# zhang-xuan1314/ABC-Net

Hardware: AMD Instinct MI355X
Metric: training images/sec (384x384, b16/GPU) (higher is better)
Workload: dtype bf16; 1 GPU; unet.py train step (pack+fwd+fused loss+bwd+allreduce+Adam), 384x384, batch 16/GPU, dropout 0.2; global_batch=16, parallelism=dp1, graph=True, device_meters=False, device_rasteriser=False, device_extraction=False, logits_stored=True

## Files before the change

abc-net_amd/_lib.py:

```python
from __future__ import annotations

import ctypes as C
import os

_HERE = os.path.dirname(os.path.abspath(__file__))
LIB_PATH = os.path.join(_HERE, "libabcnet_hip.so")

F32, BF16, FP8 = 0, 1, 2
MAX_TAPS = 49
OMEGA_RAW, OMEGA_PEAKS = 0, 1

vp, i32, u32, i64, f32, f64 = C.c_void_p, C.c_int32, C.c_uint32, C.c_int64, C.c_float, C.c_double


class ActSrc(C.Structure):
    _fields_ = [("x", vp), ("scale", vp), ("shift", vp), ("slope", vp), ("Hx", i32), ("Wx", i32), ("ldx", i32),
                ("pool", i32), ("drop_p", f32), ("drop_seed", u32), ("planar", i32), ("ctot", i32), ("drop_salt", vp)]


class ConvDesc(C.Structure):
    _fields_ = [("src", ActSrc), ("w", vp), ("bias", vp), ("y", vp), ("stats", vp),
                ("dtype_in", i32), ("dtype_c", i32), ("dtype_out", i32),
                ("B", i32), ("Hin", i32), ("Win", i32), ("cin_off", i32), ("Cin", i32), ("Hg", i32), ("Wg", i32),
                ("Hout", i32), ("Wout", i32), ("ldy", i32), ("cout_off", i32), ("Cout", i32), ("Cout_pad", i32),
                ("stride", i32), ("om", i32), ("oy0", i32), ("ox0", i32), ("ntaps", i32),
                ("tap_dy", C.c_int8 * MAX_TAPS), ("tap_dx", C.c_int8 * MAX_TAPS), ("stats_rows", i32), ("accumulate", i32),
                ("planar_out", i32), ("ctot_out", i32), ("out_act", i32), ("out_slope", f32), ("pool_y", vp), ("ld_pool", i32),
                ("stem_x", vp), ("stem_w", vp), ("stem_scale", vp), ("stem_bias", vp), ("stem_slope", f32),
                ("out_scale", vp), ("out_quant", vp), ("out_quant_stride", i32), ("heads_epi", vp),
                ("actbwd_y", vp), ("actbwd_ld", i32), ("actbwd_coff", i32), ("actbwd_scale", vp), ("actbwd_shift", vp), ("actbwd_slope", vp),
                ("actbwd_mean", vp), ("actbwd_invstd", vp), ("head_aux", vp), ("head_aux_mode", i32)]


class HeadsEpi(C.Structure):
    _fields_ = [("w2", vp), ("bias", vp), ("oscale", vp), ("y", vp), ("Cout", i32), ("Cout_pad", i32)]


class PackDesc(C.Structure):
    _fields_ = [("w", vp), ("dst", vp), ("mode", i32), ("dtype_c", i32), ("Cout", i32), ("Cin", i32), ("kh", i32),
                ("kw", i32), ("py", i32), ("px", i32), ("rows_pad", i32), ("red_pad", i32), ("red_total", i32),
                ("red_off", i32), ("ck", i32), ("rows_total", i32), ("rows_off", i32), ("layout", i32), ("row_scale", vp)]


class BnFwdDesc(C.Structure):
    _fields_ = [("partial", vp), ("nblk", i32), ("C", i32), ("count", f64), ("rows", i32), ("gamma", vp), ("beta", vp),
                ("scale", vp), ("shift", vp), ("mean", vp), ("invstd", vp), ("running_mean", vp), ("running_var", vp),
                ("num_batches_tracked", vp), ("eps", f32), ("momentum", f32)]


class ActBwdDesc(C.Structure):
    _fields_ = [("y_raw", vp), ("ld_y", i32), ("dA_same", vp), ("ld_same", i32), ("dA_pool", vp), ("ld_pool", i32),
                ("g", vp), ("ld_g", i32), ("partial", vp), ("scale", vp), ("shift", vp), ("slope", vp), ("mean", vp),
                ("invstd", vp), ("dtype", i32), ("B", i32), ("H", i32), ("W", i32), ("C", i32), ("cy_off", i32),
                ("csame_off", i32), ("cpool_off", i32), ("drop_p", f32), ("drop_seed", u32), ("drop_ld", i32), ("drop_salt", vp)]


class BnBwdDesc(C.Structure):
    _fields_ = [("partial", vp), ("nblk", i32), ("C", i32), ("count", f64), ("gamma", vp), ("invstd", vp),
                ("dgamma", vp), ("dbeta", vp), ("k1", vp), ("k2", vp), ("gscale", vp),
                ("mean", vp), ("ca", vp), ("cb", vp), ("cc", vp), ("in_scale", vp)]


class BnApplyDesc(C.Structure):
    _fields_ = [("g", vp), ("ld_g", i32), ("y_raw", vp), ("ld_y", i32), ("cy_off", i32), ("mean", vp), ("invstd", vp),
                ("k1", vp), ("k2", vp), ("gscale", vp), ("dtype", i32), ("C", i32), ("npix", i64), ("out", vp), ("ld_out", i32)]


class WgradDesc(C.Structure):
    _fields_ = [("p", ActSrc), ("q", ActSrc), ("partial", vp), ("dtype_p", i32), ("dtype_q", i32), ("dtype_c", i32),
                ("B", i32), ("Hg", i32), ("Wg", i32), ("Hq", i32), ("Wq", i32), ("cp_off", i32), ("Ca", i32),
                ("cq_off", i32), ("Cb", i32), ("stride", i32), ("ntaps", i32), ("nsplit", i32),
                ("tap_dy", C.c_int8 * MAX_TAPS), ("tap_dx", C.c_int8 * MAX_TAPS),
                ("p2", vp), ("ld_p2", i32), ("cp2_off", i32), ("p_dual", i32), ("p_out", vp), ("ld_pout", i32),
                ("rowsum_partial", vp)]


class WgradReduceDesc(C.Structure):
    _fields_ = [("partial", vp), ("nsplit", i32), ("ntaps", i32), ("Ca", i32), ("Cb", i32), ("Ca_pad", i32),
                ("Cb_pad", i32), ("dw", vp), ("accumulate", i32)]


class LossDesc(C.Structure):
    _fields_ = [("logits", vp * 8), ("dlogits", vp * 8), ("t_atom", vp), ("t_types", vp), ("t_charges", vp),
                ("t_hs", vp), ("t_bond", vp), ("t_btypes", vp), ("t_rho", vp), ("t_omega", vp), ("B", i32), ("h", i32),
                ("w", i32), ("partial", vp)]


class LossFinDesc(C.Structure):
    _fields_ = [("partial", vp), ("nblk", i32), ("s", vp), ("ds", vp), ("out", vp), ("chan_scale", vp), ("nchan", i32),
                ("chan_off", i32 * 8), ("head_c", i32 * 8), ("grad_scale", f32)]


class AdamDesc(C.Structure):
    _fields_ = [("p", vp), ("g", vp), ("m", vp), ("v", vp), ("n", i64), ("step", vp), ("lr", f32), ("beta1", f32),
                ("beta2", f32), ("eps", f32), ("weight_decay", f32), ("grad_scale", f32)]


class LossScaleDesc(C.Structure):
    _fields_ = [("dlogits", vp * 8), ("n", i64 * 8), ("head_scale", vp), ("ds", vp), ("grad_out", vp)]


ADAM_MAX_CLASSES = 32


class AdamSeg(C.Structure):
    _fields_ = [("p", vp), ("g", vp), ("m", vp), ("v", vp), ("n", i64), ("first_chunk", i64), ("cls", i32), ("pad_", i32)]


class AdamClass(C.Structure):
    _fields_ = [("step_size", f32), ("bc2_sqrt", f32), ("beta1", f32), ("beta2", f32), ("eps", f32), ("weight_decay", f32),
                ("pad_", f32 * 2)]


class AdamMultiDesc(C.Structure):
    _fields_ = [("segs", vp), ("nseg", i32), ("nclass", i32), ("chunk_total", i64), ("cls", AdamClass * ADAM_MAX_CLASSES)]


class NmsDesc(C.Structure):
    _fields_ = [("atom", vp), ("bond", vp), ("rho", vp), ("omega", vp), ("B", i32), ("h", i32), ("w", i32),
                ("n_omega", i32), ("atom_mask", vp), ("bond_mask", vp), ("rho_abs", vp), ("omega_mask", vp)]


class CbamChannelDesc(C.Structure):
    _fields_ = [("partial", vp), ("tiles_per_img", i32), ("B", i32), ("C", i32), ("mid", i32), ("HW", f64), ("scale", vp),
                ("shift", vp), ("w1", vp), ("b1", vp), ("w2", vp), ("b2", vp), ("ca", vp), ("avgz", vp), ("maxz", vp),
                ("hid_avg", vp), ("hid_max", vp), ("dw1", vp), ("db1", vp), ("dw2", vp), ("db2", vp), ("d_avgz", vp),
                ("d_maxz", vp), ("work", vp), ("ext", vp), ("first", vp)]


class CbamPixDesc(C.Structure):
    _fields_ = [("y", vp), ("ld_y", i32), ("cy_off", i32), ("scale", vp), ("shift", vp), ("mean", vp), ("invstd", vp),
                ("ca", vp), ("maxz", vp), ("d_avgz", vp), ("d_maxz", vp), ("sa", vp), ("st", vp), ("amax", vp), ("du", vp),
                ("dst", vp), ("res", vp), ("ld_res", i32), ("cres_off", i32), ("res_pool", i32), ("out", vp), ("ld_out", i32),
                ("cout_off", i32), ("d_same", vp), ("ld_same", i32), ("csame_off", i32), ("d_pool", vp), ("ld_pool", i32),
                ("cpool_off", i32), ("g", vp), ("ld_g", i32), ("dz", vp), ("ld_dz", i32), ("partial", vp), ("dtype", i32),
                ("B", i32), ("H", i32), ("W", i32), ("C", i32), ("ext", vp), ("first", vp)]


class CbamConv7Desc(C.Structure):
    _fields_ = [("st", vp), ("w7", vp), ("b7", vp), ("sa", vp), ("du", vp), ("dst", vp), ("dw_partial", vp), ("dw7", vp),
                ("db7", vp), ("B", i32), ("H", i32), ("W", i32)]


class MetricsDesc(C.Structure):
    _fields_ = [("logits", vp * 8), ("t_atom", vp), ("t_types", vp), ("t_charges", vp), ("t_hs", vp), ("t_bond", vp),
                ("t_btypes", vp), ("t_rho", vp), ("t_omega", vp), ("B", i32), ("h", i32), ("w", i32), ("peaks", vp),
                ("partial", vp), ("totals", vp), ("last", vp)]


class ExtractDesc(C.Structure):
    _fields_ = [("atom_mask", vp), ("bond_mask", vp), ("types", vp), ("charges", vp), ("hs", vp), ("btypes", vp), ("rho", vp),
                ("omega", vp), ("B", i32), ("h", i32), ("w", i32), ("cap_atoms", i32), ("cap_bonds", i32), ("counts", vp),
                ("atoms", vp), ("bonds", vp), ("bond_rho", vp), ("work", vp), ("work_masks", vp), ("btype_idx", vp),
                ("omega_rule", i32)]


class RasterDesc(C.Structure):
    _fields_ = [("t_atom", vp), ("t_types", vp), ("t_charges", vp), ("t_hs", vp), ("t_bond", vp), ("t_btypes", vp), ("t_rho", vp),
                ("t_omega", vp), ("B", i32), ("h", i32), ("w", i32), ("max_atoms", i32), ("max_bonds", i32), ("atoms", vp),
                ("n_atoms", vp), ("bonds", vp), ("n_bonds", vp), ("rho", vp), ("group_flags", vp), ("prev_atoms", vp), ("prev_bonds", vp),
                ("prev_rho", vp), ("prev_counts", vp), ("incremental", i32)]


class HeadsFusedDesc(C.Structure):
    _fields_ = [("feat", vp), ("ld", i32), ("scale", vp), ("shift", vp), ("slope", vp), ("mean", vp), ("invstd", vp),
                ("drop_p", f32), ("drop_seed", u32), ("drop_salt", vp), ("w2", vp * 8), ("b2", vp * 8), ("w2_pack", vp),
                ("logits", vp * 8), ("t_atom", vp), ("t_types", vp), ("t_charges", vp), ("t_hs", vp), ("t_bond", vp),
                ("t_btypes", vp), ("t_rho", vp), ("t_omega", vp), ("dl", vp), ("g", vp), ("bn_partial", vp), ("loss_partial", vp),
                ("B", i32), ("h", i32), ("w", i32), ("chan_scale", vp), ("chan_off", i32 * 8), ("dw2", vp * 8), ("db2", vp * 8),
                ("wgrad_work", vp), ("keep_mask", vp), ("target_flags", vp), ("zero_bytes", vp)]


class ConvTDesc(C.Structure):
    _fields_ = [("src", ActSrc), ("w", vp), ("bias", vp), ("y", vp), ("dtype", i32), ("B", i32), ("Hin", i32), ("Win", i32), ("cin_off", i32),
                ("Cin", i32), ("Hout", i32), ("Wout", i32), ("ldy", i32), ("cout_off", i32), ("Cout", i32), ("Cout_pad", i32)]


class ImageDesc(C.Structure):
    _fields_ = [("out", vp), ("src", vp), ("src_stride", i64), ("src_pitch", i32), ("src_max_h", i32), ("params", vp),
                ("params_host", vp), ("B", i32), ("S", i32), ("mode", i32), ("test_max_ink", i32)]


class AssembleDesc(C.Structure):
    _fields_ = [("counts", vp), ("atoms", vp), ("bonds", vp), ("bond_rho", vp), ("trig", vp), ("B", i32), ("cap_atoms", i32),
                ("cap_bonds", i32), ("cap_mol_bonds", i32), ("mol_counts", vp), ("mol_atoms", vp), ("mol_bonds", vp), ("mol_implh", vp),
                ("work", vp)]


class EvalDesc(C.Structure):
    _fields_ = [("atom_mask", vp), ("bond_mask", vp), ("omega_mask", vp), ("rho_abs", vp), ("types", vp), ("charges", vp), ("hs", vp),
                ("btypes", vp), ("btype_idx", vp), ("t_atom", vp), ("t_types", vp), ("t_charges", vp), ("t_hs", vp), ("t_bond", vp),
                ("t_btypes", vp), ("t_rho", vp), ("t_omega", vp), ("n_valid", vp), ("B", i32), ("h", i32), ("w", i32), ("partial", vp),
                ("counts_last", vp), ("counts_totals", vp), ("meters_last", vp), ("meters_totals", vp)]


class GraphScoreDesc(C.Structure):
    _fields_ = [("mol_counts", vp), ("mol_atoms", vp), ("mol_bonds", vp), ("rec_atoms", vp), ("rec_bonds", vp), ("rec_counts", vp),
                ("n_valid", vp), ("B", i32), ("cap_atoms", i32), ("cap_mol_bonds", i32), ("max_atoms", i32), ("max_bonds", i32),
                ("radius", i32), ("rows", vp), ("totals", vp)]


class GraphSimilarityDesc(C.Structure):
    _fields_ = [("mol_counts", vp), ("mol_atoms", vp), ("mol_bonds", vp), ("rec_atoms", vp), ("rec_bonds", vp), ("rec_counts", vp),
                ("n_valid", vp), ("B", i32), ("cap_atoms", i32), ("cap_mol_bonds", i32), ("max_atoms", i32), ("max_bonds", i32),
                ("rows", vp), ("totals", vp), ("ids_out", vp)]


class GraphIdentityDesc(C.Structure):
    _fields_ = [("mol_counts", vp), ("mol_atoms", vp), ("mol_bonds", vp), ("rec_atoms", vp), ("rec_bonds", vp), ("rec_counts", vp),
                ("n_valid", vp), ("B", i32), ("cap_atoms", i32), ("cap_mol_bonds", i32), ("max_atoms", i32), ("max_bonds", i32),
                ("max_tries", i32), ("max_rounds", i32), ("rows", vp), ("totals", vp), ("map_out", vp)]


class MolBlockDesc(C.Structure):
    _fields_ = [("mol_counts", vp), ("mol_atoms", vp), ("mol_bonds", vp), ("mol_implh", vp), ("B", i32), ("cap_atoms", i32),
                ("cap_mol_bonds", i32), ("text", vp), ("index", vp), ("work", vp), ("cap_text", i64)]


class ScanDesc(C.Structure):
    _fields_ = [("out", vp), ("src", vp), ("src_stride", i64), ("src_pitch", i32), ("src_max_h", i32), ("params", vp),
                ("params_host", vp), ("B", i32), ("S", i32), ("margin", i32), ("cover_q8", i32), ("polarity", i32), ("hist", vp),
                ("box", vp), ("geom", vp)]


class ScanCleanDesc(C.Structure):
    _fields_ = [("scratch", vp), ("stats", vp), ("labels_out", vp), ("keep_out", vp), ("cell", i32), ("min_ink", i32),
                ("keep_q8", i32)]


class StrokeDesc(C.Structure):
    _fields_ = [("src", vp), ("dst", vp), ("B", i32), ("S", i32), ("drop_isolated", i32), ("max_iter", i32), ("radius", i32),
                ("skip_stride", i32), ("skip", vp), ("stats", vp)]


EVAL_NCOUNT = 301
GRAPH_SCORE_COLUMNS = ("counted", "none", "truncated", "exact", "atoms_equal", "bonds_equal", "atoms_true", "atoms_pred",
                       "atoms_located", "atoms_matched", "bonds_true", "bonds_pred", "bonds_paired", "bonds_matched")
GRAPH_SIM_COLUMNS = ("counted", "none", "truncated", "size_equal", "refine_equal", "dice_one", "atoms_pred", "atoms_true",
                     "envs_pred", "envs_true", "envs_common", "dice_q20")
GRAPH_SIM_IDS = 2048
GRAPH_IDENT_COLUMNS = ("counted", "none", "truncated", "size_equal", "same", "different", "undecided", "levels", "tries",
                       "backtracks", "rounds")
IDENT_DEFAULT_TRIES, IDENT_DEFAULT_ROUNDS = 4096, 16384
IMG_TRAIN, IMG_TEST = 0, 1
IMG_NPARAM = 10
SCAN_NPARAM = 2
SCAN_DARK, SCAN_LIGHT, SCAN_AUTO = 0, 1, 2
SCAN_CONSTANT, SCAN_BAD_PARAMS = 1, 2
SCAN_NBOX = 8
SCAN_GEOM_COLUMNS = ("thr", "inverted", "status", "y0", "x0", "bh", "bw", "rows", "cols", "ddx", "ddy", "ink")
SCAN_NO_COMPONENT, SCAN_CLEAN_FAILED = 4, 8
SCAN_CLEAN_CELLS = (8, 16, 32, 64)
SCAN_CLEAN_COLUMNS = ("components", "kept", "ink_kept", "ink_dropped", "heaviest", "occupied_cells")
STROKE_UNTIL_STABLE = -1
STROKE_MAX_SIZE = 1024
STROKE_STAT_COLUMNS = ("iterations", "converged", "ink_in", "ink_out", "skipped")
MOL_EMPTY, MOL_TRUNCATED = 1, 2
MAX_CAP_ATOMS, MAX_BOND_PEAKS, MAX_SCORE_RECORD, MAX_SIM_ATOMS = 2048, 4096, 1024, 512
TEXT_BAD_ROW, TEXT_OVERFLOW = 4, 8


_STRUCTS = [ActSrc, ConvDesc, PackDesc, BnFwdDesc, ActBwdDesc, BnBwdDesc, BnApplyDesc, WgradDesc, WgradReduceDesc,
            LossDesc, LossFinDesc, AdamDesc, NmsDesc, CbamChannelDesc, CbamPixDesc, CbamConv7Desc, MetricsDesc, ExtractDesc, RasterDesc,
            HeadsFusedDesc, HeadsEpi, ConvTDesc, LossScaleDesc, AdamSeg, AdamClass, AdamMultiDesc, ImageDesc, AssembleDesc]

SELF_SIZED = [(EvalDesc, "abc_eval_desc_size"), (GraphScoreDesc, "abc_graph_score_desc_size"),
              (GraphSimilarityDesc, "abc_graph_similarity_desc_size"), (MolBlockDesc, "abc_molblock_desc_size"),
              (ScanDesc, "abc_scan_desc_size")]
SELF_SIZED_SINCE = [(StrokeDesc, "abc_stroke_desc_size"), (GraphIdentityDesc, "abc_graph_identity_desc_size"),
                    (ScanCleanDesc, "abc_scan_clean_desc_size")]

P = C.POINTER
SYMBOLS = {
    "abc_conv_stat_blocks": (C.c_int, [P(ConvDesc)]),
    "abc_convt_fused_ok": (C.c_int, [P(ConvTDesc)]),
    "abc_convt_fused_fwd": (C.c_int, [P(ConvTDesc), vp]),
    "abc_conv_actbwd_ok": (C.c_int, [P(ConvDesc)]),
    "abc_conv_fwd_batch": (C.c_int, [P(ConvDesc), C.c_int32, C.c_void_p]),
    "abc_conv_batch_ok": (C.c_int, [P(ConvDesc), C.c_int32]),
    "abc_conv_variant": (C.c_int, [vp]),
    "abc_conv_weight_layout": (C.c_int, [vp]),
    "abc_conv_fwd": (C.c_int, [P(ConvDesc), vp]),
    "abc_conv_chunk": (C.c_int, [C.c_int, C.c_int]),
    "abc_heads_batch": (C.c_int, [vp, i32, i32, vp]),
    "abc_heads_fused_pack_bytes": (i64, []),
    "abc_heads_fused_chunks": (C.c_int, [P(HeadsFusedDesc)]),
    "abc_heads_fused_loss_blocks": (C.c_int, [P(HeadsFusedDesc)]),
    "abc_heads_fused_dl_elems": (i64, [P(HeadsFusedDesc)]),
    "abc_heads_fused_wgrad_floats": (i64, [P(HeadsFusedDesc)]),
    "abc_heads_fused_rows": (C.c_int, [i32]),
    "abc_heads_fused_chan_of_row": (C.c_int, [i32, i32]),
    "abc_heads_fused_pack": (C.c_int, [P(HeadsFusedDesc), vp]),
    "abc_heads_fused_fwd_bwd": (C.c_int, [P(HeadsFusedDesc), vp]),
    "abc_heads_fused_wgrad": (C.c_int, [P(HeadsFusedDesc), vp]),
    "abc_conv_tile": (C.c_int, [P(ConvDesc), P(i32), P(i32), P(i32)]),
    "abc_pack_conv_weights": (C.c_int, [P(PackDesc), vp]),
    "abc_pack_item_bytes": (C.c_int, []),
    "abc_pack_item_fill": (i64, [vp, P(PackDesc), i64]),
    "abc_pack_batch": (C.c_int, [vp, i32, i64, vp]),
    "abc_bn_finalize_fwd": (C.c_int, [P(BnFwdDesc), vp]),
    "abc_bn_finalize_fwd_batch": (C.c_int, [vp, i32, i32, vp]),
    "abc_bn_finalize_bwd_batch": (C.c_int, [vp, i32, i32, vp]),
    "abc_bn_eval_coeffs": (C.c_int, [vp, vp, vp, vp, vp, vp, i32, f32, vp]),
    "abc_bn_eval_fold": (C.c_int, [vp, vp, vp, vp, vp, vp, vp, i32, f32, vp]),
    "abc_act_bwd_blocks": (C.c_int, [P(ActBwdDesc)]),
    "abc_act_bwd": (C.c_int, [P(ActBwdDesc), vp]),
    "abc_bn_finalize_bwd": (C.c_int, [P(BnBwdDesc), vp]),
    "abc_bn_apply_bwd": (C.c_int, [P(BnApplyDesc), vp]),
    "abc_wgrad_fuses_apply": (C.c_int, [vp]),
    "abc_wgrad_rowsum_ok": (C.c_int, [vp]),
    "abc_wgrad_pads": (C.c_int, [P(WgradDesc), P(i32), P(i32)]),
    "abc_wgrad_blocks": (C.c_int, [P(WgradDesc)]),
    "abc_wgrad_tile": (C.c_int, [P(WgradDesc), P(i32), P(i32)]),
    "abc_wgrad_route_info": (C.c_int, [P(WgradDesc), P(i32)]),
    "abc_wgrad": (C.c_int, [P(WgradDesc), vp]),
    "abc_wgrad_reduce": (C.c_int, [P(WgradReduceDesc), vp]),
    "abc_wgrad_reduce_bn_bwd": (C.c_int, [P(WgradReduceDesc), P(BnBwdDesc), vp]),
    "abc_wgrad_heads_batch": (C.c_int, [vp, i32, vp]),
    "abc_wgrad_reduce_batch": (C.c_int, [vp, i32, vp]),
    "abc_colsum_blocks": (C.c_int, [i64]),
    "abc_colsum": (C.c_int, [vp, i32, i64, i32, i32, i32, vp, vp, vp, vp]),
    "abc_colsum_w1": (C.c_int, [vp, i32, i64, i32, i32, i32, vp, vp, vp, vp, vp]),
    "abc_loss_blocks": (C.c_int, [P(LossDesc)]),
# ... 126 lines not shown
```

abc-net_amd/csrc/heads_fused.hip:

```cpp
#include "common.hpp"
#include "../../include/abcnet_hip.h"
#include "capi_util.hpp"
#include "loss_math.hpp"
#include "heads_fused.hpp"
#include <stdlib.h>

namespace {

struct HFHead {
    const bf16* w2f;
    const bf16* w2t;
    const float* biasp;
    float* logits;
    bf16* dlb;
    uint2* keep;
};

struct HFK {
    const bf16* y1;
    const float *sc, *sh, *sl, *mean, *invstd;
    bf16* g;
    int ld;
    float drop_p;
    uint32_t drop_seed, drop_thr;
    const uint32_t* drop_salt;
    const float *t_atom, *t_types, *t_charges, *t_hs, *t_bond, *t_btypes;
    const double *t_rho, *t_omega;
    const uint32_t* tflags;
    const char* tzero;
    float* bnpart;
    float* dwsmall;
    double* losspart;
    int HW, nchunk;
    HFHead hd[HF_NH];
};

constexpr int TROW = 32 * 2 + 16;
constexpr int HROW = 64 * 2 + 16;
constexpr int WV_BIAS = 2560, WV_CF = 5120, WV_DN = 8704;
constexpr int WV_AIMG = 7680, AROW = 128 * 2 + 16;
constexpr int WV = 16384;
constexpr int LDS_BSUM = 4 * WV;
constexpr int LDS_LSUM = LDS_BSUM + 4 * 2 * 2 * 128 * 4;
constexpr int HF_LDS = LDS_LSUM + 4 * 16 * 8;

struct Ctx {
    int lane, r, h, wave, chunk, b, yx, nslice;
    uint32_t pix, pix0;
    char* ot;
    float* dnl;
    float* wsum;
    float dscale;
    uint32_t dseed;
};

typedef __attribute__((address_space(3))) bf16x4 lds_bf16x4_f;
__device__ inline bf16x8 tr_read8f(const char* b0, const char* b1) {
    bf16x4 lo = __builtin_amdgcn_ds_read_tr16_b64_v4bf16((lds_bf16x4_f*)b0);
    bf16x4 hi = __builtin_amdgcn_ds_read_tr16_b64_v4bf16((lds_bf16x4_f*)b1);
    return __builtin_shufflevector(lo, hi, 0, 1, 2, 3, 4, 5, 6, 7);
}

__device__ inline void lds_sync() { asm volatile("s_waitcnt lgkmcnt(0)" ::: "memory"); }

__device__ inline double wave_sum_d(double v) {
#pragma unroll
    for (int o = 32; o > 0; o >>= 1) v += __shfl_xor(v, o);
    return v;
}

template <int HEAD>
__device__ inline void small_head_wgrad(const HFK& a, const Ctx& c, const bf16x8* fb) {
    constexpr int CH = hf_ch(HEAD);
    const int r = c.r, h = c.h, lane = c.lane;
    char* img = c.ot + WV_AIMG;
#pragma unroll
    for (int kk = 0; kk < 8; ++kk) *(bf16x8*)(img + r * AROW + (16 * kk + 8 * h) * 2) = fb[kk];
    __syncthreads();
    const int trow = 8 * h + ((lane & 15) >> 2), tcol = 16 * ((lane >> 4) & 1) + 4 * (lane & 3);
    f32x16 aw, ab;
#pragma unroll
    for (int k = 0; k < 16; ++k) { aw[k] = 0.f; ab[k] = 0.f; }
    bf16x8 ones;
#pragma unroll
    for (int j = 0; j < 8; ++j) ones[j] = (bf16)1.0f;
#pragma unroll
    for (int w2 = 0; w2 < 4; ++w2) {
        const char* tw = c.ot + (w2 - c.wave) * WV;
#pragma unroll
        for (int s2 = 0; s2 < 2; ++s2) {
            const bf16x8 fa2 = *(const bf16x8*)(tw + r * TROW + (16 * s2 + 8 * h) * 2);
            const char* q0 = tw + WV_AIMG + (16 * s2 + trow) * AROW + (32 * c.wave + tcol) * 2;
            const bf16x8 fb2 = tr_read8f(q0, q0 + 4 * AROW);
            aw = __builtin_amdgcn_mfma_f32_32x32x16_bf16(fa2, fb2, aw, 0, 0, 0);
            ab = __builtin_amdgcn_mfma_f32_32x32x16_bf16(fa2, ones, ab, 0, 0, 0);
        }
    }
    if (h == 0) {
        float* dst = a.dwsmall + ((size_t)c.chunk * HF_SMALL_ROWS + hf_small_row0(HEAD)) * 129;
#pragma unroll
        for (int k = 0; k < CH; ++k) {
            dst[k * 129 + 32 * c.wave + r] = aw[k];
            if (c.wave == 0 && r == 0) dst[k * 129 + 128] = ab[k];
        }
    }
    __syncthreads();
}

template <int HEAD>
__device__ inline void run_head_skip(const HFK& a, Ctx& c, double* lsum) {
    static_assert(HEAD == 1 || HEAD == 2 || HEAD == 3 || HEAD == 5, "softmax heads");
    constexpr int CH = hf_ch(HEAD), NT = hf_tiles(HEAD), CPAD = NT * 32;
    const HFHead& hd = a.hd[HEAD];
    const int slice = 128 * HEAD;
    const int r = c.r, h = c.h, lane = c.lane;
    const uint32_t lch = HEAD >= 5 ? 30u * h : 0u;
    const uint32_t loff = ((uint32_t)(c.b * CH) + lch) * (uint32_t)a.HW + (uint32_t)c.yx;
    auto at4w = [&](float* base, int chu) -> float* { return (float*)((char*)(base + (size_t)chu * a.HW) + 4u * loff); };
    float* cf = (float*)(c.ot + WV_CF);
    float* bl = (float*)(c.ot + WV_BIAS);
    const uint32_t e0 = c.pix * (uint32_t)a.ld + slice + 8 * h;
    const bool st_logits = hd.logits != nullptr;
    const u32x4 z4 = {0u, 0u, 0u, 0u};
    bf16x8 fb[8];
    uint32_t kbits[2] = {0u, 0u};
    if (st_logits || (HEAD >= 5 && hd.keep != nullptr)) {
        u32x4 raw[8];
#pragma unroll
        for (int kk = 0; kk < 8; ++kk) raw[kk] = *(const u32x4*)(a.y1 + e0 + 16 * kk);
        {
            const int ch = slice + 2 * lane;
            const float2 v0 = *(const float2*)(a.sc + ch), v1 = *(const float2*)(a.sh + ch), v2 = *(const float2*)(a.sl + ch);
            *(float2*)(cf + 0 * 128 + 2 * lane) = v0; *(float2*)(cf + 1 * 128 + 2 * lane) = v1; *(float2*)(cf + 2 * 128 + 2 * lane) = v2;
#pragma unroll
            for (int i = 0; i < (CPAD + 63) / 64; ++i)
                if (lane + 64 * i < CPAD) bl[lane + 64 * i] = hd.biasp[lane + 64 * i];
        }
        lds_sync();
#pragma unroll
        for (int kk = 0; kk < 8; ++kk) {
            float v[8], sc[8], sh[8], sl[8];
            const int cc = 16 * kk + 8 * h;
            LoadVec<float, 8>::ld(cf + cc, sc); LoadVec<float, 8>::ld(cf + 128 + cc, sh); LoadVec<float, 8>::ld(cf + 256 + cc, sl);
#pragma unroll
            for (int j = 0; j < 4; ++j) { v[2 * j] = __uint_as_float(raw[kk][j] << 16); v[2 * j + 1] = __uint_as_float(raw[kk][j] & 0xFFFF0000u); }
#pragma unroll
            for (int j = 0; j < 8; ++j) {
                const float y = fmaf(v[j], sc[j], sh[j]);
                const bool keep = a.drop_p > 0.f ? abc_drop_hash24(e0 + 16 * kk + j, c.dseed) >= a.drop_thr : true;
                kbits[kk >> 2] |= (keep ? 1u : 0u) << (8 * (kk & 3) + j);
                v[j] = keep ? fmaxf(y, sl[j] * y) * c.dscale : 0.f;
            }
            fb[kk] = pack_frag<bf16>(v);
        }
    } else {
#pragma unroll
        for (int kk = 0; kk < 8; ++kk) fb[kk] = __builtin_bit_cast(bf16x8, z4);
    }
    if (st_logits) {
        bf16x8 fa[8];
        auto load_fa = [&](int mt) {
#pragma unroll
            for (int kk = 0; kk < 8; ++kk)
                fa[kk] = *(const bf16x8*)((const char*)(hd.w2f + (size_t)((kk >> 1) * CPAD + 32 * mt) * 32 + 16 * (kk & 1)) + (uint32_t)(r * 64 + h * 16));
        };
        load_fa(0);
#pragma unroll 1
        for (int mt = 0; mt < NT; ++mt) {
            f32x16 acc;
#pragma unroll
            for (int q = 0; q < 4; ++q) {
                const f32x4 b4 = *(const f32x4*)(bl + 32 * mt + 8 * q + 4 * h);
#pragma unroll
                for (int j = 0; j < 4; ++j) acc[4 * q + j] = b4[j];
            }
#pragma unroll
            for (int kk = 0; kk < 8; ++kk) acc = __builtin_amdgcn_mfma_f32_32x32x16_bf16(fa[kk], fb[kk], acc, 0, 0, 0);
            __builtin_amdgcn_sched_barrier(0);
            load_fa(mt + 1 < NT ? mt + 1 : mt);
            __builtin_amdgcn_sched_barrier(0);
            if constexpr (HEAD == 5) {
#pragma unroll
                for (int gi = 0; gi < 2; ++gi)
#pragma unroll
                    for (int k = 0; k < 6; ++k) *at4w(hd.logits, k * 60 + 2 * mt + gi) = acc[8 * gi + k];
            } else if (h == 0) {
#pragma unroll
                for (int k = 0; k < CH; ++k) *at4w(hd.logits, k) = acc[k];
            }
        }
    }
#pragma unroll 1
    for (int mt = 0; mt < NT; ++mt)
#pragma unroll
        for (int j = 0; j < 2; ++j) {
            const int q = lane + 64 * j, row = q >> 2, part = q & 3;
            *(u32x4*)((char*)(hd.dlb + ((size_t)c.chunk * CPAD + 32 * mt) * 128) + (uint32_t)((row * 128 + 32 * c.wave + part * 8) * 2)) = z4;
        }
    if constexpr (HEAD == 5) {
#pragma unroll
        for (int j = 0; j < 30; ++j) c.dnl[j * 64 + lane] = 0.f;
    } else {
#pragma unroll
        for (int j = 0; j < 2; ++j) {
            const int q = lane + 64 * j, row = q >> 2, part = q & 3;
            *(u32x4*)(c.ot + row * TROW + part * 16) = z4;
        }
        lds_sync();
        small_head_wgrad<HEAD>(a, c, fb);
    }
    {
        const int sg = lane & 7, pg = lane >> 3;
#pragma unroll
        for (int half = 0; half < 2; ++half)
#pragma unroll
            for (int it = 0; it < 4; ++it)
                *(u32x4*)(a.g + (size_t)(c.pix0 + it * 8 + pg) * a.ld + slice + 64 * half + sg * 8) = z4;
        float* ws = c.wsum + c.nslice * 256;
#pragma unroll
        for (int i = 0; i < 4; ++i) ws[lane + 64 * i] = 0.f;
    }
    if constexpr (HEAD >= 5) {
        if (hd.keep != nullptr) hd.keep[2u * c.pix + h] = make_uint2(kbits[0], kbits[1]);
    }
    c.nslice += 1;
    if (lane == 0) {
        lsum[HEAD] = 0.0;
        lsum[8 + HEAD] = 0.0;
        if (HEAD == 5) lsum[8 + 6] = 0.0;
    }
}

template <int HEAD>
__device__ inline void run_head(const HFK& a, Ctx& c, double* lsum) {
    double num = 0.0, den = 0.0;
    constexpr int CH = hf_ch(HEAD), NT = hf_tiles(HEAD), CPAD = NT * 32;
    const HFHead& hd = a.hd[HEAD];
    const int slice = 128 * HEAD;
    const int r = c.r, h = c.h, lane = c.lane;
    const uint32_t lch = HEAD >= 5 ? 30u * h : 0u;
    const uint32_t loff = ((uint32_t)(c.b * CH) + lch) * (uint32_t)a.HW + (uint32_t)c.yx;
    const uint32_t tword = a.tflags ? (uint32_t)__builtin_amdgcn_readfirstlane((int)a.tflags[c.pix0 >> 5]) : 0xFFFFFFFFu;
    const bool tz = !((tword >> (HEAD == 6 ? 5 : HEAD)) & 1u);
    if constexpr (HEAD == 1 || HEAD == 2 || HEAD == 3 || HEAD == 5) {
        if (tz) { run_head_skip<HEAD>(a, c, lsum); return; }
    }
    const size_t thw = tz ? (size_t)0 : (size_t)a.HW;
    const uint32_t tloff = tz ? (uint32_t)lane : loff;
    auto tbase4 = [&](const float* base) -> const float* { return tz ? (const float*)a.tzero : base; };
    auto tbase8 = [&](const double* base) -> const double* { return tz ? (const double*)a.tzero : base; };
    auto at4 = [&](const float* base, int chu) -> const float* { return (const float*)((const char*)(tbase4(base) + (size_t)chu * thw) + 4u * tloff); };
    auto at4w = [&](float* base, int chu) -> float* { return (float*)((char*)(base + (size_t)chu * a.HW) + 4u * loff); };
    auto at8 = [&](const double* base, int chu) -> const double* { return (const double*)((const char*)(tbase8(base) + (size_t)chu * thw) + 8u * tloff); };
    float* cf = (float*)(c.ot + WV_CF);
    float* bl = (float*)(c.ot + WV_BIAS);
    const uint32_t e0 = c.pix * (uint32_t)a.ld + slice + 8 * h;

    u32x4 raw[8];
#pragma unroll
    for (int kk = 0; kk < 8; ++kk) raw[kk] = *(const u32x4*)(a.y1 + e0 + 16 * kk);
    {
        const int ch = slice + 2 * lane;
        const float2 v0 = *(const float2*)(a.sc + ch), v1 = *(const float2*)(a.sh + ch), v2 = *(const float2*)(a.sl + ch),
                     v3 = *(const float2*)(a.mean + ch), v4 = *(const float2*)(a.invstd + ch);
        *(float2*)(cf + 0 * 128 + 2 * lane) = v0; *(float2*)(cf + 1 * 128 + 2 * lane) = v1; *(float2*)(cf + 2 * 128 + 2 * lane) = v2;
        *(float2*)(cf + 3 * 128 + 2 * lane) = v3; *(float2*)(cf + 4 * 128 + 2 * lane) = v4;
#pragma unroll
        for (int i = 0; i < (CPAD + 63) / 64; ++i)
            if (lane + 64 * i < CPAD) bl[lane + 64 * i] = hd.biasp[lane + 64 * i];
    }
    bf16x8 fa[8];
    auto load_fa = [&](int mt) {
#pragma unroll
        for (int kk = 0; kk < 8; ++kk)
            fa[kk] = *(const bf16x8*)((const char*)(hd.w2f + (size_t)((kk >> 1) * CPAD + 32 * mt) * 32 + 16 * (kk & 1)) + (uint32_t)(r * 64 + h * 16));
    };
    float tn[HEAD == 5 ? 12 : 1];
    auto load_t5 = [&](int mt) {
        if constexpr (HEAD == 5) {
#pragma unroll
            for (int gi = 0; gi < 2; ++gi)
#pragma unroll
                for (int k = 0; k < 6; ++k) tn[6 * gi + k] = *at4(a.t_btypes, k * 60 + 2 * mt + gi);
        }
    };
    constexpr bool PIPE = HEAD == 5;
    if constexpr (PIPE) { load_fa(0); load_t5(0); }

    double wpix = 0.0;
    if constexpr (HEAD == 7) {
        double wp = 0.0;
#pragma unroll 6
        for (int j = 0; j < 30; ++j) {
            const double t = *at8(a.t_omega, j);
            wp += t;
            c.dnl[j * 64 + lane] = (float)t;
        }
        wpix = wp + __shfl_xor(wp, 32);
        den = (h == 0) ? wpix : 0.0;
    }

    lds_sync();
    bf16x8 fb[8];
    uint32_t kbits[2] = {0u, 0u}, pbits[2] = {0u, 0u};
#pragma unroll
    for (int kk = 0; kk < 8; ++kk) {
        float v[8], sc[8], sh[8], sl[8];
        const int cc = 16 * kk + 8 * h;
        LoadVec<float, 8>::ld(cf + cc, sc); LoadVec<float, 8>::ld(cf + 128 + cc, sh); LoadVec<float, 8>::ld(cf + 256 + cc, sl);
#pragma unroll
        for (int j = 0; j < 4; ++j) { v[2 * j] = __uint_as_float(raw[kk][j] << 16); v[2 * j + 1] = __uint_as_float(raw[kk][j] & 0xFFFF0000u); }
#pragma unroll
        for (int j = 0; j < 8; ++j) {
            const float y = fmaf(v[j], sc[j], sh[j]);
            const bool keep = a.drop_p > 0.f ? abc_drop_hash24(e0 + 16 * kk + j, c.dseed) >= a.drop_thr : true;
            const int bit = 8 * (kk & 3) + j;
            kbits[kk >> 2] |= (keep ? 1u : 0u) << bit;
            pbits[kk >> 2] |= (y > 0.f ? 1u : 0u) << bit;
            v[j] = keep ? fmaxf(y, sl[j] * y) * c.dscale : 0.f;
        }
        fb[kk] = pack_frag<bf16>(v);
    }
    asm volatile("" : "+v"(kbits[0]), "+v"(kbits[1]), "+v"(pbits[0]), "+v"(pbits[1]));

    const bool st_logits = hd.logits != nullptr;
    f32x16 accD[4];
#pragma unroll
    for (int mi = 0; mi < 4; ++mi)
#pragma unroll
        for (int k = 0; k < 16; ++k) accD[mi][k] = 0.f;
    bf16x8 wt[8], bqp[2];
    auto dgrad_mfma = [&]() {
#pragma unroll
        for (int u = 0; u < 2; ++u)
#pragma unroll
            for (int mi = 0; mi < 4; ++mi) accD[mi] = __builtin_amdgcn_mfma_f32_32x32x16_bf16(wt[4 * u + mi], bqp[u], accD[mi], 0, 0, 0);
    };

#pragma unroll 1
    for (int mt = 0; mt < NT; ++mt) {
        if (PIPE && mt > 0) dgrad_mfma();
        if constexpr (!PIPE) load_fa(mt);
        f32x16 acc;
#pragma unroll
        for (int q = 0; q < 4; ++q) {
            const f32x4 b4 = *(const f32x4*)(bl + 32 * mt + 8 * q + 4 * h);
#pragma unroll
            for (int j = 0; j < 4; ++j) acc[4 * q + j] = b4[j];
        }
#pragma unroll
        for (int kk = 0; kk < 8; ++kk) acc = __builtin_amdgcn_mfma_f32_32x32x16_bf16(fa[kk], fb[kk], acc, 0, 0, 0);
        float v[16], dlv[16];
#pragma unroll
        for (int k = 0; k < 16; ++k) { v[k] = acc[k]; dlv[k] = 0.f; }
        if constexpr (HEAD == 5) {
#pragma unroll
            for (int gi = 0; gi < 2; ++gi) {
                float z[6], t[6], dz[6], dn = 0.f;
#pragma unroll
                for (int k = 0; k < 6; ++k) { z[k] = v[8 * gi + k]; t[k] = tn[6 * gi + k]; }
                num += (double)class_focal<6, true>(z, t, nullptr, dz, &dn);
                den += (double)dn;
                c.dnl[(2 * mt + gi) * 64 + lane] = dn;
#pragma unroll
                for (int k = 0; k < 6; ++k) dlv[8 * gi + k] = dz[k];
            }
            __builtin_amdgcn_sched_barrier(0);
            {
                const int mtn = mt + 1 < NT ? mt + 1 : mt;
                load_fa(mtn);
#pragma unroll
                for (int u = 0; u < 2; ++u)
#pragma unroll
                    for (int mi = 0; mi < 4; ++mi)
                        wt[4 * u + mi] = *(const bf16x8*)((const char*)(hd.w2t + (size_t)((2 * mt + u) * 128 + 32 * mi) * 16) + (uint32_t)(r * 32 + h * 16));
                load_t5(mtn);
            }
            __builtin_amdgcn_sched_barrier(0);
            if (st_logits) {
#pragma unroll
                for (int gi = 0; gi < 2; ++gi)
#pragma unroll
                    for (int k = 0; k < 6; ++k) *at4w(hd.logits, k * 60 + 2 * mt + gi) = v[8 * gi + k];
            }
        } else if constexpr (HEAD == 6) {
#pragma unroll
            for (int k = 0; k < 16; ++k) {
                const int j = 16 * mt + k;
                if (j < 30) {
                    const float zr = v[k];
                    const double tr = *at8(a.t_rho, j);
                    if (st_logits) *at4w(hd.logits, j) = zr;
                    const float dn = c.dnl[j * 64 + lane];
                    const double diff = (double)fabsf(zr) - tr;
                    num += fabs(diff) * (double)dn;
                    const float sg = (diff > 0.0) ? 1.f : ((diff < 0.0) ? -1.f : 0.f);
                    const float sz = (zr > 0.f) ? 1.f : ((zr < 0.f) ? -1.f : 0.f);
                    dlv[k] = sg * sz * dn;
                }
                if ((k & 3) == 3) __builtin_amdgcn_sched_barrier(0);
            }
        } else if constexpr (HEAD == 7) {
#pragma unroll
            for (int k = 0; k < 16; ++k) {
                const int j = 16 * mt + k;
                if (j < 30) {
                    if (st_logits) *at4w(hd.logits, j) = v[k];
                    float dz;
                    num += (double)center_focal<true>(v[k], c.dnl[j * 64 + lane], (float)wpix, &dz);
                    dlv[k] = dz;
                }
                if ((k & 1) == 1) __builtin_amdgcn_sched_barrier(0);
            }
        } else if (h == 0) {
            if constexpr (HEAD == 0 || HEAD == 4) {
                const float t = *at4(HEAD == 0 ? a.t_atom : a.t_bond, 0);
                if (st_logits) *at4w(hd.logits, 0) = v[0];
                float dz;
                num += (double)center_focal<true>(v[0], t, 1.f, &dz);
                den += (t == 1.f) ? 1.0 : 0.0;
                dlv[0] = dz;
            } else {
                const float* tg = HEAD == 1 ? a.t_types : (HEAD == 2 ? a.t_charges : a.t_hs);
                float z[CH], t[CH], dz[CH], dn = 0.f;
#pragma unroll
                for (int k = 0; k < CH; ++k) t[k] = *at4(tg, k);
#pragma unroll
                for (int k = 0; k < CH; ++k) {
                    z[k] = v[k];
                    if (st_logits) *at4w(hd.logits, k) = z[k];
                }
                num += (double)class_focal<CH, true>(z, t, HEAD == 1 ? c_type_w : nullptr, dz, &dn);
                den += (double)dn;
#pragma unroll
                for (int k = 0; k < CH; ++k) dlv[k] = dz[k];
            }
        }

        bqp[0] = pack_frag<bf16>(dlv);
        bqp[1] = pack_frag<bf16>(dlv + 8);
        char* tl = c.ot;
#pragma unroll
        for (int k = 0; k < 16; ++k) *(bf16*)(tl + ((k & 3) + 8 * (k >> 2) + 4 * h) * TROW + r * 2) = bqp[k >> 3][k & 7];
        lds_sync();
#pragma unroll
        for (int j = 0; j < 2; ++j) {
            const int q = lane + 64 * j, row = q >> 2, part = q & 3;
            const u32x4 t = *(const u32x4*)(tl + row * TROW + part * 16);
            *(u32x4*)((char*)(hd.dlb + ((size_t)c.chunk * CPAD + 32 * mt) * 128) + (uint32_t)((row * 128 + 32 * c.wave + part * 8) * 2)) = t;
        }
        lds_sync();
        if constexpr (!PIPE) {
#pragma unroll
            for (int u = 0; u < 2; ++u)
#pragma unroll
                for (int mi = 0; mi < 4; ++mi)
                    wt[4 * u + mi] = *(const bf16x8*)((const char*)(hd.w2t + (size_t)((2 * mt + u) * 128 + 32 * mi) * 16) + (uint32_t)(r * 32 + h * 16));
            if (mt + 1 < NT) dgrad_mfma();
        }
    }
#pragma unroll
    for (int kk = 0; kk < 8; ++kk) raw[kk] = *(const u32x4*)(a.y1 + e0 + 16 * kk);
    dgrad_mfma();

    if constexpr (HEAD < 5) small_head_wgrad<HEAD>(a, c, fb);

    char* ot = c.ot;
    const int sg = lane & 7, pg = lane >> 3;
    float* ws = c.wsum + c.nslice * 256;
#pragma unroll
    for (int half = 0; half < 2; ++half) {
        float gv[2][16], gx[2][16];
#pragma unroll
        for (int m2 = 0; m2 < 2; ++m2) {
            const int mi = 2 * half + m2;
#pragma unroll
            for (int k8 = 0; k8 < 2; ++k8) {
                const int kk = 2 * mi + k8, cc = 16 * kk + 8 * h;
                float sl[8], mu[8], is[8];
                LoadVec<float, 8>::ld(cf + 256 + cc, sl); LoadVec<float, 8>::ld(cf + 384 + cc, mu); LoadVec<float, 8>::ld(cf + 512 + cc, is);
                const uint32_t kb = kbits[kk >> 2] >> (8 * (kk & 3)), pb = pbits[kk >> 2] >> (8 * (kk & 3));
#pragma unroll
                for (int j = 0; j < 8; ++j) {
                    const uint32_t w = raw[kk][j >> 1];
                    const float x = __uint_as_float((j & 1) ? (w & 0xFFFF0000u) : (w << 16));
                    const float m1 = ((pb >> j) & 1u) ? c.dscale : sl[j] * c.dscale;
                    const float gg = ((kb >> j) & 1u) ? accD[mi][8 * k8 + j] * m1 : 0.f;
                    gv[m2][8 * k8 + j] = gg;
                    gx[m2][8 * k8 + j] = gg * ((x - mu[j]) * is[j]);
                }
            }
        }
#pragma unroll
        for (int pass = 0; pass < 2; ++pass) {
#pragma unroll
            for (int m2 = 0; m2 < 2; ++m2)
#pragma unroll
                for (int q = 0; q < 4; ++q) {
                    bf16x4 o;
#pragma unroll
                    for (int j = 0; j < 4; ++j) o[j] = (bf16)(pass ? gx[m2][4 * q + j] : gv[m2][4 * q + j]);
                    *(bf16x4*)(ot + r * HROW + (32 * m2 + 16 * (q >> 1) + 8 * h + 4 * (q & 1)) * 2) = o;
                }
            lds_sync();
            float acc8[8];
#pragma unroll
            for (int j = 0; j < 8; ++j) acc8[j] = 0.f;
#pragma unroll
            for (int it = 0; it < 4; ++it) {
                const int px = it * 8 + pg;
                const bf16x8 tv = *(const bf16x8*)(ot + px * HROW + sg * 16);
                if (pass == 0) *(bf16x8*)(a.g + (size_t)(c.pix0 + px) * a.ld + slice + 64 * half + sg * 8) = tv;
#pragma unroll
                for (int j = 0; j < 8; ++j) acc8[j] += (float)tv[j];
            }
            lds_sync();
#pragma unroll
            for (int j = 0; j < 8; ++j) {
                acc8[j] += __shfl_xor(acc8[j], 8); acc8[j] += __shfl_xor(acc8[j], 16); acc8[j] += __shfl_xor(acc8[j], 32);
            }
            if (lane < 8) {
#pragma unroll
                for (int j = 0; j < 8; ++j) ws[pass * 128 + 64 * half + sg * 8 + j] = acc8[j];
            }
        }
    }
    if constexpr (HEAD >= 5) {
        if (hd.keep != nullptr) hd.keep[2u * c.pix + h] = make_uint2(kbits[0], kbits[1]);
    }
    c.nslice += 1;
    {
        const double s1 = wave_sum_d(num), s2 = wave_sum_d(den);
        if (lane == 0) {
            lsum[HEAD] = s1;
            if (HEAD != 6) lsum[8 + HEAD] = s2;
            if (HEAD == 5) lsum[8 + 6] = s2;
        }
    }
}

__global__ __launch_bounds__(256, 2) void heads_fused_kernel(const HFK a) {
    extern __shared__ __attribute__((aligned(16))) char smem[];
    Ctx c;
    c.lane = threadIdx.x & 63; c.wave = threadIdx.x >> 6;
    c.r = c.lane & 31; c.h = c.lane >> 5;
    c.chunk = blockIdx.x;
    c.pix0 = (uint32_t)c.chunk * 128u + 32u * c.wave;
    c.pix = c.pix0 + c.r;
    c.b = (int)(c.pix0 / (uint32_t)a.HW);
    c.yx = (int)(c.pix - (uint32_t)c.b * (uint32_t)a.HW);
    c.ot = smem + c.wave * WV;
    c.dnl = (float*)(smem + c.wave * WV + WV_DN);
    const int group = blockIdx.y;
    c.wsum = (float*)(smem + LDS_BSUM) + c.wave * 512;
    c.nslice = 0;
    c.dscale = a.drop_p > 0.f ? 1.0f / (1.0f - a.drop_p) : 1.0f;
    c.dseed = a.drop_seed + ((a.drop_p > 0.f && a.drop_salt) ? *a.drop_salt : 0u);
    double* ls = (double*)(smem + LDS_LSUM);
    double* lsum = ls + c.wave * 16;
    if (c.lane < 16) lsum[c.lane] = 0.0;
    lds_sync();
    switch (group) {
        case 0: run_head<5>(a, c, lsum); run_head<6>(a, c, lsum); break;
        case 1: run_head<7>(a, c, lsum); break;
        case 2: run_head<0>(a, c, lsum); break;
        case 3: run_head<1>(a, c, lsum); break;
        case 4: run_head<2>(a, c, lsum); break;
        case 5: run_head<3>(a, c, lsum); break;
        default: run_head<4>(a, c, lsum); break;
    }
    __syncthreads();
    if (threadIdx.x < 16) {
        const int i = threadIdx.x & 7;
        const bool mine = group == 0 ? (i == 5 || i == 6) : (group == 1 ? i == 7 : i == group - 2);
        if (mine)
            a.losspart[(size_t)c.chunk * 16 + threadIdx.x] = (ls[threadIdx.x] + ls[16 + threadIdx.x]) + (ls[32 + threadIdx.x] + ls[48 + threadIdx.x]);
    }
    {
        const int nsl = group == 0 ? 2 : 1;
        const float* base = (const float*)(smem + LDS_BSUM);
        for (int i = threadIdx.x; i < nsl * 256; i += 256) {
            const int sl_i = i >> 8, row = (i >> 7) & 1, ch = i & 127;
            const float s = (base[i] + base[512 + i]) + (base[1024 + i] + base[1536 + i]);
            const int head = group == 0 ? 5 + sl_i : (group == 1 ? 7 : group - 2);
            a.bnpart[((size_t)c.chunk * 2 + row) * a.ld + 128 * head + ch] = s;
        }
    }
}

struct HFPackK {
    const float* w2[HF_NH];
    const float* b2[HF_NH];
    bf16* pack;
};

__global__ __launch_bounds__(256) void heads_fused_pack_kernel(const HFPackK a) {
    const int head = blockIdx.y;
    const int cpad = hf_tiles(head) * 32;
    const int idx = blockIdx.x * 256 + threadIdx.x;
    if (idx >= cpad * 128) return;
    char* base = (char*)a.pack + hf_pack_off(head);
    bf16* w2f = (bf16*)base;
    bf16* w2t = (bf16*)(base + (size_t)cpad * 256);
    float* biasp = (float*)(base + (size_t)cpad * 512);
    const float* w = a.w2[head];
    {
        const int within = idx & 31, m = (idx >> 5) % cpad, chunk = idx / (32 * cpad);
        const int ch = hf_chan_of_row(head, m);
        w2f[idx] = (bf16)(ch >= 0 ? w[ch * 128 + chunk * 32 + within] : 0.f);
    }
    {
        const int j = idx & 7, h = (idx >> 3) & 1, mrow = (idx >> 4) & 127, s = idx >> 11;
        const int ci = (mrow & ~12) | ((mrow & 4) << 1) | ((mrow & 8) >> 1);
        const int k = 8 * (s & 1) + j;
        const int m = 32 * (s >> 1) + (k & 3) + 8 * (k >> 2) + 4 * h;
        const int ch = hf_chan_of_row(head, m);
        w2t[idx] = (bf16)(ch >= 0 ? w[ch * 128 + ci] : 0.f);
    }
    if (idx < cpad) {
        const int ch = hf_chan_of_row(head, idx);
        biasp[idx] = ch >= 0 ? a.b2[head][ch] : 0.f;
    }
}

static int hf_check(const abc_heads_fused_desc* d) {
    if (d->B < 1 || d->h < 1 || d->w < 1 || (d->h * d->w) % 128) return abc_fail(ABC_EINVAL, "heads_fused: the map must hold whole 128-pixel chunks");
    if (d->ld < 128 * HF_NH || d->ld % 8) return abc_fail(ABC_EINVAL, "heads_fused: feature stride");
    if ((int64_t)d->B * d->h * d->w * d->ld >= (int64_t(1) << 32) || (int64_t)d->B * d->h * d->w * 360 >= (int64_t(1) << 31))
        return abc_fail(ABC_EUNSUPPORTED, "heads_fused: 32-bit element offsets");
    return ABC_OK;
}

}

extern "C" int64_t abc_heads_fused_pack_bytes(void) { return hf_pack_off(HF_NH); }
extern "C" int abc_heads_fused_chunks(const abc_heads_fused_desc* d) { return d->B * d->h * d->w / 128; }
extern "C" int abc_heads_fused_loss_blocks(const abc_heads_fused_desc* d) { return abc_heads_fused_chunks(d); }
extern "C" int64_t abc_heads_fused_dl_elems(const abc_heads_fused_desc* d) { return (int64_t)abc_heads_fused_chunks(d) * hf_rows_total() * 128; }
extern "C" int abc_heads_fused_rows(int32_t head) { return head >= 0 && head < HF_NH ? hf_tiles(head) * 32 : -1; }
extern "C" int abc_heads_fused_chan_of_row(int32_t head, int32_t row) {
    return (head >= 0 && head < HF_NH && row >= 0 && row < hf_tiles(head) * 32) ? hf_chan_of_row(head, row) : -1;
}

extern "C" int abc_heads_fused_pack(const abc_heads_fused_desc* d, abc_stream_t stream) {
    HFPackK k;
    for (int i = 0; i < HF_NH; ++i) { k.w2[i] = d->w2[i]; k.b2[i] = d->b2[i]; }
    k.pack = (bf16*)d->w2_pack;
    hipLaunchKernelGGL(heads_fused_pack_kernel, dim3(abc_cdiv(480 * 128, 256), HF_NH), dim3(256), 0, (hipStream_t)stream, k);
    return abc_check_launch("heads_fused_pack");
}

extern "C" int abc_heads_fused_fwd_bwd(const abc_heads_fused_desc* d, abc_stream_t stream) {
    if (int rc = hf_check(d)) return rc;
    HFK k;
    k.y1 = (const bf16*)d->feat; k.sc = d->scale; k.sh = d->shift; k.sl = d->slope; k.mean = d->mean; k.invstd = d->invstd;
    k.g = (bf16*)d->g; k.ld = d->ld;
    k.drop_p = d->drop_p; k.drop_seed = d->drop_seed; k.drop_salt = d->drop_salt; k.drop_thr = abc_drop_threshold(d->drop_p);
    k.t_atom = d->t_atom; k.t_types = d->t_types; k.t_charges = d->t_charges; k.t_hs = d->t_hs; k.t_bond = d->t_bond;
    k.t_btypes = d->t_btypes; k.t_rho = d->t_rho; k.t_omega = d->t_omega;
    if ((d->target_flags != nullptr) != (d->zero_bytes != nullptr)) return abc_fail(ABC_EINVAL, "heads_fused: target_flags and zero_bytes go together");
    k.tflags = d->target_flags; k.tzero = (const char*)d->zero_bytes;
    k.bnpart = d->bn_partial; k.losspart = d->loss_partial; k.dwsmall = d->wgrad_work;
    k.HW = d->h * d->w; k.nchunk = abc_heads_fused_chunks(d);
    size_t row0 = 0;
    for (int i = 0; i < HF_NH; ++i) {
        const int cpad = hf_tiles(i) * 32;
        char* base = (char*)d->w2_pack + hf_pack_off(i);
        k.hd[i].w2f = (const bf16*)base;
        k.hd[i].w2t = (const bf16*)(base + (size_t)cpad * 256);
        k.hd[i].biasp = (const float*)(base + (size_t)cpad * 512);
        k.hd[i].logits = d->logits[i];
        k.hd[i].dlb = (bf16*)d->dl + row0 * (size_t)k.nchunk * 128;
        k.hd[i].keep = (i >= 5 && d->keep_mask != nullptr && d->drop_p > 0.f) ? (uint2*)d->keep_mask + (size_t)(i - 5) * 2 * d->B * d->h * d->w : nullptr;
        row0 += cpad;
    }
    static unsigned long long lds_ok = 0;
    if (int rc = abc_allow_lds((const void*)heads_fused_kernel, HF_LDS, &lds_ok)) return rc;
    hipLaunchKernelGGL(heads_fused_kernel, dim3(k.nchunk, HF_GROUPS), dim3(256), HF_LDS, (hipStream_t)stream, k);
    return abc_check_launch("heads_fused_fwd_bwd");
}
```

abc-net_amd/csrc/wgrad_heads.hip:

```cpp
#include "wgrad_parts.hpp"
#include "capi_util.hpp"
#include "heads_fused.hpp"

namespace {

struct HeadK {
    const float* dl;
    const float *psc, *psh, *psl;
    const void* q;
    const float *qsc, *qsh, *qsl;
    float* partial;
    float* rowsum;
    int HW, hc, ldq, cq_off, nchunks, nsplit, mtiles, Ca_pad;
    float drop_p;
    uint32_t drop_seed;
    const uint32_t* drop_salt;
    unsigned bytesP, bytesQ;
    int cpad_blk;
    const uint8_t* keep;
};

constexpr int HQ_PSW = 320;
constexpr int HP_RSW = 272;
constexpr int HEAD_PBUF = 128 * HP_RSW, HEAD_QBUF = 128 * HQ_PSW;
constexpr int HEAD_LDS = 2 * (HEAD_PBUF + HEAD_QBUF) + 3 * 128 * 4;

template <bool BLK>
__device__ inline void head_wgrad_body(const HeadK& a, const int split, const int mg) {
    extern __shared__ __attribute__((aligned(16))) char smem[];
    const int tid = threadIdx.x, lane = tid & 63, wave = tid >> 6;
    const int r = lane & 31, h = lane >> 5;
    const int mi = wave & 3, nh = wave >> 2;
    if (split >= a.nsplit || mg * 4 >= a.mtiles) return;
    const int mt = mg * 4 + mi;
    const bool active = __builtin_amdgcn_readfirstlane(mt) < a.mtiles;
    const bool ptrans = a.psc != nullptr;
    const int c0 = (int)((long long)split * a.nchunks / a.nsplit), c1 = (int)((long long)(split + 1) * a.nchunks / a.nsplit);

    const __amdgpu_buffer_rsrc_t rsP = abc_make_rsrc(a.dl, a.bytesP), rsQ = abc_make_rsrc(a.q, a.bytesQ);
    const int part = tid & 15, pix0 = tid >> 4;
    const bool qtrans = a.qsc != nullptr;
    float* sCoef = (float*)(smem + 2 * (HEAD_PBUF + HEAD_QBUF));
    if (qtrans && tid < 128) {
        sCoef[tid] = a.qsc[a.cq_off + tid]; sCoef[128 + tid] = a.qsh[a.cq_off + tid]; sCoef[256 + tid] = a.qsl[a.cq_off + tid];
    }
    const int pseg = tid & 31, prow0 = tid >> 5;
    float psc[8], psh[8], psl[8], rsum[8];
#pragma unroll
    for (int i = 0; i < 8; ++i) {
        const int co = mg * 128 + prow0 + 16 * i;
        const bool ok = co < a.hc;
        psc[i] = (ok && ptrans) ? a.psc[co] : 1.f; psh[i] = (ok && ptrans) ? a.psh[co] : 0.f; psl[i] = (ok && ptrans) ? a.psl[co] : 1.f;
        rsum[i] = 0.f;
    }
    __syncthreads();
    const float dscale = a.drop_p > 0.f ? 1.0f / (1.0f - a.drop_p) : 1.0f;
    const uint32_t dseed = a.drop_seed + ((a.drop_p > 0.f && a.drop_salt) ? *a.drop_salt : 0u);
    u32x4 qreg0[4], preg0[8], qreg1[4], preg1[8];
    const bool kmask = BLK && a.keep != nullptr && a.drop_p > 0.f;
    const __amdgpu_buffer_rsrc_t rsK = abc_make_rsrc(kmask ? a.keep : (const uint8_t*)a.q, kmask ? (unsigned)a.nchunks * 2048u : 0u);
    const unsigned kbyte = (unsigned)((part & 1) * 8 + (part >> 1));
    const int CPI = a.HW / 128;
    auto issue = [&](int c, u32x4 (&qreg)[4], u32x4 (&preg)[8]) {
        const bool live = c < c1;
        const int b = c / CPI, pp0 = (c - b * CPI) * 128;
        const unsigned qoff = live ? (unsigned)(((unsigned)(c * 128 + pix0) * (unsigned)a.ldq + (unsigned)(a.cq_off + part * 8)) * 2u) : 0x80000000u;
#pragma unroll
        for (int i = 0; i < 4; ++i) qreg[i] = __builtin_amdgcn_raw_buffer_load_b128(rsQ, live ? qoff + (unsigned)(i * 32 * a.ldq * 2) : qoff, 0, 0);
        if constexpr (BLK) {
            if (kmask) {
                const unsigned koff = live ? (unsigned)(c * 128 + pix0) * 16u + kbyte : 0x80000000u;
#pragma unroll
                for (int i = 0; i < 4; ++i) preg[4][i] = (unsigned)__builtin_amdgcn_raw_buffer_load_b8(rsK, live ? koff + (unsigned)(i * 32 * 16) : koff, 0, 0);
            }
#pragma unroll
            for (int i = 0; i < 4; ++i) {
                const int row = mg * 128 + (tid >> 4) + 32 * i;
                const unsigned poff = (live && row < a.cpad_blk) ? (unsigned)((((unsigned)c * (unsigned)a.cpad_blk + (unsigned)row) * 128u + 8u * (tid & 15)) * 2u) : 0x80000000u;
                preg[i] = __builtin_amdgcn_raw_buffer_load_b128(rsP, poff, 0, 0);
            }
        } else {
#pragma unroll
        for (int i = 0; i < 8; ++i) {
            const int co = mg * 128 + prow0 + 16 * i;
            const unsigned poff = (live && co < a.hc) ? (unsigned)((((unsigned)(b * a.hc + co)) * (unsigned)a.HW + (unsigned)(pp0 + 4 * pseg)) * 4u) : 0x80000000u;
            preg[i] = __builtin_amdgcn_raw_buffer_load_b128(rsP, poff, 0, 0);
        }
        }
    };
    auto commit = [&](int c, char* sP, char* sQ, const u32x4 (&qreg)[4], const u32x4 (&preg)[8]) {
        float qsc[8], qsh[8], qsl[8];
        if (qtrans) {
#pragma unroll
            for (int j = 0; j < 8; ++j) { qsc[j] = sCoef[part * 8 + j]; qsh[j] = sCoef[128 + part * 8 + j]; qsl[j] = sCoef[256 + part * 8 + j]; }
        }
#pragma unroll
        for (int i = 0; i < 4; ++i) {
            const int pix = pix0 + 32 * i;
            const uint32_t eoff = (uint32_t)(c * 128 + pix) * (uint32_t)a.ldq + (uint32_t)(a.cq_off + part * 8);
            float v[8];
#pragma unroll
            for (int j = 0; j < 4; ++j) { v[2 * j] = __uint_as_float(qreg[i][j] << 16); v[2 * j + 1] = __uint_as_float(qreg[i][j] & 0xFFFF0000u); }
            if (qtrans) {
#pragma unroll
                for (int j = 0; j < 8; ++j) v[j] = abc_act(v[j], qsc[j], qsh[j], qsl[j]);
            }
            if (BLK && kmask) {
                const unsigned kb = preg[4][i];
#pragma unroll
                for (int j = 0; j < 8; ++j) v[j] = ((kb >> j) & 1u) ? v[j] * dscale : 0.f;
            } else if (a.drop_p > 0.f) {
#pragma unroll
                for (int j = 0; j < 8; ++j) v[j] = abc_drop_keep(eoff + j, dseed, a.drop_p) ? v[j] * dscale : 0.f;
            }
            *(bf16x8*)(sQ + pix * HQ_PSW + part * 16) = pack_frag<bf16>(v);
        }
        if constexpr (BLK) {
#pragma unroll
            for (int i = 0; i < 4; ++i) {
                float f = 0.f;
#pragma unroll
                for (int j = 0; j < 4; ++j) f += __uint_as_float(preg[i][j] << 16) + __uint_as_float(preg[i][j] & 0xFFFF0000u);
                rsum[i] += f;
                *(u32x4*)(sP + ((tid >> 4) + 32 * i) * HP_RSW + (tid & 15) * 16) = preg[i];
            }
            return;
        }
#pragma unroll
        for (int i = 0; i < 8; ++i) {
            const bool ok = mg * 128 + prow0 + 16 * i < a.hc;
            float f[4];
#pragma unroll
            for (int j = 0; j < 4; ++j) {
                f[j] = __uint_as_float(preg[i][j]);
                if (ptrans) f[j] = abc_act(f[j], psc[i], psh[i], psl[i]);
                if (!ok) f[j] = 0.f;
            }
            rsum[i] += (f[0] + f[1]) + (f[2] + f[3]);
            bf16x4 o;
#pragma unroll
            for (int j = 0; j < 4; ++j) o[j] = (bf16)f[j];
            *(bf16x4*)(sP + (prow0 + 16 * i) * HP_RSW + pseg * 8) = o;
        }
    };

    f32x16 acc[2];
#pragma unroll
    for (int j = 0; j < 2; ++j)
#pragma unroll
        for (int k = 0; k < 16; ++k) acc[j][k] = 0.f;

    const int sub = 16 * ((lane >> 4) & 1) + 4 * (lane & 3);
    const int qlane = (64 * h + ((lane & 15) >> 2)) * HQ_PSW + sub * 2;
    const int plane = (mi * 32 + r) * HP_RSW + (64 * h) * 2;

    auto compute = [&](const char* sP, const char* sQ) {
#pragma unroll
        for (int kk = 0; kk < 8; ++kk) {
            const bf16x8 fa = *(const bf16x8*)(sP + plane + kk * 16);
            const char* qb = sQ + qlane + kk * 8 * HQ_PSW + nh * 128;
            const bf16x8 fb0 = tr_read8(qb, qb + 4 * HQ_PSW);
            const bf16x8 fb1 = tr_read8(qb + 64, qb + 64 + 4 * HQ_PSW);
            acc[0] = __builtin_amdgcn_mfma_f32_32x32x16_bf16(fa, fb0, acc[0], 0, 0, 0);
            acc[1] = __builtin_amdgcn_mfma_f32_32x32x16_bf16(fa, fb1, acc[1], 0, 0, 0);
        }
    };

    constexpr int BUF = HEAD_PBUF + HEAD_QBUF;
    char* const b0 = smem;
    char* const b1 = smem + BUF;
    issue(c0, qreg0, preg0);
    issue(c0 + 1, qreg1, preg1);
    if (c0 < c1) commit(c0, b0, b0 + HEAD_PBUF, qreg0, preg0);
    __syncthreads();
    for (int c = c0; c < c1; c += 2) {
        issue(c + 2, qreg0, preg0);
        if (active) compute(b0, b0 + HEAD_PBUF);
        if (c + 1 < c1) commit(c + 1, b1, b1 + HEAD_PBUF, qreg1, preg1);
        __syncthreads();
        if (c + 1 < c1) {
            issue(c + 3, qreg1, preg1);
            if (active) compute(b1, b1 + HEAD_PBUF);
            if (c + 2 < c1) commit(c + 2, b0, b0 + HEAD_PBUF, qreg0, preg0);
            __syncthreads();
        }
    }
    if (BLK && a.rowsum != nullptr) {
#pragma unroll
        for (int i = 0; i < 4; ++i) {
            float v = rsum[i];
#pragma unroll
            for (int m = 8; m >= 1; m >>= 1) v += __shfl_xor(v, m);
            const int row = mg * 128 + (tid >> 4) + 32 * i;
            if ((tid & 15) == 0 && row < a.Ca_pad) a.rowsum[(size_t)split * a.Ca_pad + row] = v;
        }
    } else if (a.rowsum != nullptr) {
#pragma unroll
        for (int i = 0; i < 8; ++i) {
            float v = rsum[i];
#pragma unroll
            for (int m = 16; m >= 1; m >>= 1) v += __shfl_xor(v, m);
            const int row = mg * 128 + prow0 + 16 * i;
            if (pseg == 0 && row < a.Ca_pad) a.rowsum[(size_t)split * a.Ca_pad + row] = v;
        }
    }
    if (active) {
#pragma unroll
        for (int j = 0; j < 2; ++j) {
            float* out = a.partial + ((size_t)split * a.Ca_pad + mt * 32) * 128 + (nh * 2 + j) * 32 + r;
#pragma unroll
            for (int k = 0; k < 16; ++k) {
                const int arow = (k & 3) + 8 * (k >> 2) + 4 * h;
                out[(size_t)arow * 128] = acc[j][k];
            }
        }
    }
}

__global__ __launch_bounds__(512, 2) void head_wgrad_kernel(const HeadK a) { head_wgrad_body<false>(a, blockIdx.x, blockIdx.y); }
struct HeadWgBatch { HeadK k[8]; int first[9]; };
__global__ __launch_bounds__(512, 2) void head_wgrad_batch_kernel(const HeadWgBatch bt) { head_wgrad_body<false>(bt.k[blockIdx.z], blockIdx.x, blockIdx.y); }
__global__ __launch_bounds__(512, 2) void head_wgrad_blocked_kernel(const HeadWgBatch bt) {
    const int id = blockIdx.x;
    int hd = 0;
    while (hd < 7 && id >= bt.first[hd + 1]) ++hd;
    const HeadK& k = bt.k[hd];
    const int units = (k.mtiles + 3) >> 2, local = id - bt.first[hd];
    head_wgrad_body<true>(k, local / units, local % units);
}

static void head_fill(HeadK& k, const abc_wgrad_desc* d) {
    k.dl = (const float*)d->p.x; k.psc = d->p.scale; k.psh = d->p.shift; k.psl = d->p.slope;
    k.q = d->q.x; k.qsc = d->q.scale; k.qsh = d->q.shift; k.qsl = d->q.slope;
    k.partial = d->partial; k.rowsum = d->rowsum_partial; k.HW = d->Hg * d->Wg; k.hc = d->Ca; k.ldq = d->q.ldx; k.cq_off = d->cq_off;
    k.nchunks = d->B * k.HW / 128; k.nsplit = d->nsplit; k.mtiles = abc_cdiv(d->Ca, 32); k.Ca_pad = k.mtiles * 32;
    k.drop_p = d->q.drop_p; k.drop_seed = d->q.drop_seed; k.drop_salt = d->q.drop_salt;
    k.bytesP = (unsigned)((int64_t)d->B * d->Ca * k.HW * 4); k.bytesQ = (unsigned)((int64_t)d->B * k.HW * d->q.ldx * 2);
    k.cpad_blk = 0; k.keep = nullptr;
}

static bool head_dims_ok(const abc_wgrad_desc* d) { return d->p.Hx == d->Hg && d->p.Wx == d->Wg && d->q.Hx == d->Hg && d->q.Wx == d->Wg; }

}

int abc_wgrad_head_ok(const abc_wgrad_desc* d) {
    if (!d->p.planar || d->dtype_p != ABC_F32 || d->dtype_q != ABC_BF16 || d->dtype_c != ABC_BF16) return 0;
    if (d->ntaps != 1 || d->tap_dy[0] != 0 || d->tap_dx[0] != 0 || d->stride != 1 || d->Cb != 128 || d->cp_off != 0) return 0;
    if (d->q.pool || d->q.planar || d->p.pool || d->p.drop_p > 0.f || (d->Hg * d->Wg) % 128) return 0;
    if (d->p.ctot != d->Ca) return 0;
    const int64_t bp = (int64_t)d->B * d->Ca * d->Hg * d->Wg * 4, bq = (int64_t)d->B * d->Hg * d->Wg * d->q.ldx * 2;
    return bp < (int64_t(1) << 31) && bq < (int64_t(1) << 31) && (d->q.ldx % 8) == 0 && (d->cq_off % 8) == 0;
}

int abc_wgrad_head_launch(const abc_wgrad_desc* d, abc_stream_t stream) {
    if (!head_dims_ok(d)) return abc_fail(ABC_EINVAL, "wgrad: dims mismatch");
    HeadK k;
    head_fill(k, d);
    static unsigned long long lds_ok = 0;
    if (int rc = abc_allow_lds((const void*)head_wgrad_kernel, 160 * 1024, &lds_ok)) return rc;
    hipLaunchKernelGGL(head_wgrad_kernel, dim3(d->nsplit, abc_cdiv(k.mtiles, 4)), dim3(512), HEAD_LDS, (hipStream_t)stream, k);
    return abc_check_launch("head_wgrad");
}

extern "C" int abc_wgrad_heads_batch(const abc_wgrad_desc* descs, int32_t n, abc_stream_t stream) {
    if (n < 1 || n > 8) return abc_fail(ABC_EINVAL, "wgrad_heads_batch: 1..8 heads");
    HeadWgBatch bt;
    int gx = 0, gy = 0;
    for (int i = 0; i < n; ++i) {
        const abc_wgrad_desc* d = descs + i;
        if (d->nsplit < 1 || d->ntaps != 1 || !abc_wgrad_head_ok(d)) return abc_fail(ABC_EUNSUPPORTED, "wgrad_heads_batch: not a heads' 1x1 weight gradient");
        if (!head_dims_ok(d)) return abc_fail(ABC_EINVAL, "wgrad: dims mismatch");
        head_fill(bt.k[i], d);
        gx = bt.k[i].nsplit > gx ? bt.k[i].nsplit : gx;
        gy = abc_cdiv(bt.k[i].mtiles, 4) > gy ? abc_cdiv(bt.k[i].mtiles, 4) : gy;
    }
    for (int i = n; i < 8; ++i) bt.k[i] = bt.k[0];
    static unsigned long long lds_ok = 0;
    if (int rc = abc_allow_lds((const void*)head_wgrad_batch_kernel, 160 * 1024, &lds_ok)) return rc;
    hipLaunchKernelGGL(head_wgrad_batch_kernel, dim3(gx, gy, n), dim3(512), HEAD_LDS, (hipStream_t)stream, bt);
    return abc_check_launch("wgrad_heads_batch");
}

static void hf_splits(int nchunk, int* nsplit) {
    double cost[HF_NH], tot = 0;
    int units[HF_NH];
    for (int i = 5; i < HF_NH; ++i) {
        units[i] = abc_cdiv(hf_tiles(i), 4);
        cost[i] = 4.0 + 1.5 * (double)hf_tiles(i) / units[i] / 4.0;
        tot += units[i] * cost[i];
    }
    for (int i = 0; i < HF_NH; ++i) {
        if (i < 5) { nsplit[i] = 0; continue; }
        int n = (int)(256.0 * cost[i] / tot);
        n = n < 1 ? 1 : n;
        nsplit[i] = n > nchunk ? nchunk : n;
    }
}

extern "C" int64_t abc_heads_fused_wgrad_floats(const abc_heads_fused_desc* d) {
    int ns[HF_NH];
    const int nchunk = d->B * d->h * d->w / 128;
    hf_splits(nchunk, ns);
    int64_t n = (int64_t)(nchunk + 16) * HF_SMALL_ROWS * 129;
    for (int i = 5; i < HF_NH; ++i) n += (int64_t)ns[i] * hf_tiles(i) * 32 * (128 + 1);
    return n;
}

struct HeadFusedRedK {
    const float* partial[HF_NH]; const float* rowsum[HF_NH];
    float* dw[HF_NH]; float* db[HF_NH];
    const float* chan_scale;
    const float* small2;
    int nsplit[HF_NH], chan_off[HF_NH];
};
__global__ __launch_bounds__(192) void head_fused_small_reduce_kernel(const float* part, int nchunk, float* out) {
    const int row = blockIdx.x, sl = blockIdx.y, c2 = threadIdx.x;
    if (c2 >= 129) return;
    const float* p = part + (size_t)row * 129 + c2;
    const size_t step = (size_t)HF_SMALL_ROWS * 129;
    float s0 = 0.f, s1 = 0.f, s2 = 0.f, s3 = 0.f;
    int k = sl;
    for (; k + 48 < nchunk; k += 64) {
        s0 += p[(size_t)k * step]; s1 += p[(size_t)(k + 16) * step]; s2 += p[(size_t)(k + 32) * step]; s3 += p[(size_t)(k + 48) * step];
    }
    for (; k < nchunk; k += 16) s0 += p[(size_t)k * step];
    out[((size_t)sl * HF_SMALL_ROWS + row) * 129 + c2] = (s0 + s1) + (s2 + s3);
}
__global__ __launch_bounds__(128) void head_fused_reduce_kernel(const HeadFusedRedK a) {
    const int head = blockIdx.y, ch = blockIdx.x, ci = threadIdx.x;
    if (ch >= hf_ch(head)) return;
    const float cs = a.chan_scale[a.chan_off[head] + ch];
    if (head < 5) {
        const float* p = a.small2 + (size_t)(hf_small_row0(head) + ch) * 129;
        for (int c2 = ci; c2 < 129; c2 += 128) {
            float s = 0.f;
#pragma unroll
            for (int k = 0; k < 16; ++k) s += p[(size_t)k * HF_SMALL_ROWS * 129 + c2];
            if (c2 < 128) a.dw[head][ch * 128 + c2] = s * cs; else a.db[head][ch] = s * cs;
        }
        return;
    }
    const int cpad = hf_tiles(head) * 32, row = hf_row_of_chan(head, ch);
    const float* p = a.partial[head] + (size_t)row * 128 + ci;
    float s0 = 0.f, s1 = 0.f;
    int k = 0;
    for (; k + 2 <= a.nsplit[head]; k += 2) { s0 += p[(size_t)k * cpad * 128]; s1 += p[(size_t)(k + 1) * cpad * 128]; }
    if (k < a.nsplit[head]) s0 += p[(size_t)k * cpad * 128];
    a.dw[head][ch * 128 + ci] = (s0 + s1) * cs;
    if (ci == 0) {
        float b = 0.f;
        for (int q = 0; q < a.nsplit[head]; ++q) b += a.rowsum[head][(size_t)q * cpad + row];
        a.db[head][ch] = b * cs;
    }
}

extern "C" int abc_heads_fused_wgrad(const abc_heads_fused_desc* d, abc_stream_t stream) {
    const int HW = d->h * d->w, nchunk = d->B * HW / 128;
    if (HW % 128 || d->ld % 8 || (int64_t)d->B * HW * d->ld * 2 >= (int64_t(1) << 31))
        return abc_fail(ABC_EUNSUPPORTED, "heads_fused_wgrad: whole 128-pixel chunks, feature buffer below 2 GB");
    int ns[HF_NH];
    hf_splits(nchunk, ns);
    HeadWgBatch bt;
    HeadFusedRedK rk;
    float* ws = d->wgrad_work + (size_t)nchunk * HF_SMALL_ROWS * 129;
    rk.small2 = ws; ws += 16 * HF_SMALL_ROWS * 129;
    size_t row0 = 0;
    for (int i = 0; i < HF_NH; ++i) {
        const int cpad = hf_tiles(i) * 32;
        rk.dw[i] = d->dw2[i]; rk.db[i] = d->db2[i]; rk.nsplit[i] = ns[i]; rk.chan_off[i] = d->chan_off[i];
        rk.partial[i] = nullptr; rk.rowsum[i] = nullptr;
        if (i >= 5) {
            HeadK& k = bt.k[i - 5];
            k.dl = (const float*)((const bf16*)d->dl + row0 * (size_t)nchunk * 128);
            k.psc = k.psh = k.psl = nullptr;
            k.q = d->feat; k.qsc = d->scale; k.qsh = d->shift; k.qsl = d->slope;
            k.partial = ws; ws += (size_t)ns[i] * cpad * 128;
            k.rowsum = ws; ws += (size_t)ns[i] * cpad;
            k.HW = HW; k.hc = hf_ch(i); k.ldq = d->ld; k.cq_off = 128 * i; k.nchunks = nchunk; k.nsplit = ns[i];
            k.mtiles = hf_tiles(i); k.Ca_pad = cpad;
            k.drop_p = d->drop_p; k.drop_seed = d->drop_seed; k.drop_salt = d->drop_salt;
            k.bytesP = (unsigned)((size_t)nchunk * cpad * 128 * 2); k.bytesQ = (unsigned)((int64_t)d->B * HW * d->ld * 2);
            k.cpad_blk = cpad;
            k.keep = d->keep_mask != nullptr ? (const uint8_t*)d->keep_mask + (size_t)(i - 5) * nchunk * 2048 : nullptr;
            if ((size_t)nchunk * cpad * 128 * 2 >= (size_t(1) << 31)) return abc_fail(ABC_EUNSUPPORTED, "heads_fused_wgrad: d(logits) block above 2 GB");
            rk.partial[i] = k.partial; rk.rowsum[i] = k.rowsum;
        }
        row0 += cpad;
    }
    for (int i = 3; i < 8; ++i) bt.k[i] = bt.k[0];
    bt.first[0] = 0;
    for (int i = 0; i < 8; ++i) bt.first[i + 1] = bt.first[i] + (i < 3 ? bt.k[i].nsplit * abc_cdiv(bt.k[i].mtiles, 4) : 0);
    rk.chan_scale = d->chan_scale;
    static unsigned long long lds_ok = 0;
    if (int rc = abc_allow_lds((const void*)head_wgrad_blocked_kernel, 160 * 1024, &lds_ok)) return rc;
    hipLaunchKernelGGL(head_wgrad_blocked_kernel, dim3(bt.first[8]), dim3(512), HEAD_LDS, (hipStream_t)stream, bt);
    if (int rc = abc_check_launch("heads_fused_wgrad")) return rc;
    hipLaunchKernelGGL(head_fused_small_reduce_kernel, dim3(HF_SMALL_ROWS, 16), dim3(192), 0, (hipStream_t)stream, (const float*)d->wgrad_work, nchunk, (float*)rk.small2);
    hipLaunchKernelGGL(head_fused_reduce_kernel, dim3(360, HF_NH), dim3(128), 0, (hipStream_t)stream, rk);
    return abc_check_launch("heads_fused_wgrad_reduce");
}
```

abc-net_amd/engine.py:

```python
from __future__ import annotations

import ctypes as C
import weakref
from typing import NamedTuple

import torch

from . import _lib as L
from . import arch

BN_EPS = 1e-5
BN_MOM = 0.1
DROP_STEP = 0x9E3779B9
def head_offsets(heads):
    offs, o = [], 0
    for h in heads:
        offs.append(o)
        o += h
    return offs


def taps_square(k):
    p = (k - 1) // 2
    return [(ky - p, kx - p) for ky in range(k) for kx in range(k)]


def taps_mirror(taps):
    return [(-dy, -dx) for dy, dx in taps]


def convT_phase_taps(py, px, crop_y=True, crop_x=True):
    def axis(p, crop):
        if crop:
            return [0] if p == 0 else [1, 0]
        return [0, -1] if p == 0 else [0]
    return [(dy, dx) for dy in axis(py, crop_y) for dx in axis(px, crop_x)]


def convT_pack_parity(p, crop):
    return p if crop else 1 - p


def convT_dgrad_taps(crop_y=True, crop_x=True):
    cy, cx = (1 if crop_y else 0), (1 if crop_x else 0)
    return [(ky - cy, kx - cx) for ky in range(3) for kx in range(3)]


TAPS_CONVT_DGRAD = convT_dgrad_taps()


class Op(NamedTuple):
    fn: object
    args: list
    what: str
    writes: tuple
    meta: dict


class Src:

    def __init__(self, t, dt, H, W, ld, coff, C, coef=None, pool=False, drop_p=0.0, drop_seed=0, producer=None, planar=False):
        self.t, self.dt, self.H, self.W, self.ld, self.coff, self.C = t, dt, H, W, ld, coff, C
        self.coef, self.pool, self.drop_p, self.drop_seed, self.producer = coef, pool, drop_p, drop_seed, producer
        self.drop_salt = None
        self.planar = planar
        self.q = None

    def lh(self):
        return (self.H // 2, self.W // 2) if self.pool else (self.H, self.W)

    def fill(self, a: L.ActSrc):
        a.x = self.t.data_ptr()
        a.planar, a.ctot = (1, self.C) if self.planar else (0, 0)
        if self.coef is not None:
            a.scale, a.shift, a.slope = (c.data_ptr() for c in self.coef)
        else:
            a.scale = a.shift = a.slope = None
        a.Hx, a.Wx, a.ldx, a.pool = self.H, self.W, self.ld, 1 if self.pool else 0
        a.drop_p, a.drop_seed = self.drop_p, self.drop_seed
        a.drop_salt = self.drop_salt.data_ptr() if (self.drop_salt is not None and self.drop_p > 0) else None


class Rec:

    def __init__(self, **kw):
        self.grad_same = None
        self.grad_pool = None
        self.__dict__.update(kw)


def set_reserved_cus(n):
    lib = L.load()
    n = (int(n) + 3) & ~3
    if n == lib.abc_get_reserved_cus():
        return n
    alive = [e for e in Engine._live]
    if alive:
        raise L.AbcNetHipError("cannot change the reserved-CU count from %d to %d: %d plan(s) built under the current value are alive "
                               "(it is a process-wide setting baked into their grids; build every Trainer / InferenceRunner of this "
                               "process with the same reserve_cus, or drop the old ones first)" % (lib.abc_get_reserved_cus(), n, len(alive)))
    L.check(lib.abc_set_reserved_cus(n), "set_reserved_cus")
    return n


class Engine:
    _live = weakref.WeakSet()

    def __init__(self, variant, in_channels, heads, params, grads, buffers, counters, layout, B, H, W, dtype, train,
                 dropout_p=0.2, device="cuda", drop_seed=0x1234ABCD, fold_bn=False, fused_heads=False, batched_heads=True, fp8=False,
                 guards=False, heads_epilogue=False, actbwd_epilogue=True, merge_reduce=True, nms_heads=False, decode=False,
                 dual_wgrad=True, fused_convt=True):
        if variant not in ("unet", "unet2"):
            raise NotImplementedError("variant %r" % variant)
        if H < 32 or W < 32:
            raise ValueError("H and W must be at least 32 (five 2x2 poolings; got %dx%d)" % (H, W))
        if in_channels < 1:
            raise ValueError("in_channels must be positive")
        self.in_channels = in_channels
        self.lib = L.load()
        self.reserved_cus = self.lib.abc_get_reserved_cus()
        self.dual_wgrad = bool(dual_wgrad)
        self.fused_convt = bool(fused_convt)
        self.variant, self.heads, self.B, self.H, self.W = variant, list(heads), B, H, W
        self.train = train
        self.fold = bool(fold_bn)
        if self.fold and (train or variant != "unet"):
            raise ValueError("fold_bn is the eval-mode graph of unet.py")
        self.fp8 = bool(fp8)
        if self.fp8 and not (self.fold and dtype == "bf16"):
            raise ValueError("fp8 is a form of the BatchNorm-folded bf16 inference graph (fold_bn=True, dtype='bf16')")
        self.fp8_recs = []
        self.hfeat_q = None
        self.fp8_calibrated = False
        self.guards = bool(guards)
        self._guarded = []
        self.heads_epilogue = bool(heads_epilogue)
        self.nms_heads = bool(nms_heads) and not train
        self.nms_rho = self.nms_omega = None
        self.decode = bool(decode) and self.nms_heads
        self.btype_idx = None
        self.actbwd_epilogue = bool(actbwd_epilogue)
        self.merge_reduce = bool(merge_reduce)
        self._pending_reduce = None
        self.dt = L.BF16 if dtype == "bf16" else L.F32
        self.tdt = torch.bfloat16 if dtype == "bf16" else torch.float32
        self.batched_heads = bool(batched_heads)
        self.want_fused_heads = bool(fused_heads) and train and dtype == "bf16" and self.batched_heads and self.heads == arch.TRAIN_HEADS
        self.hf = None
        self.dev = device
        self.params, self.grads, self.buffers, self.counters = params, grads, buffers, counters
        self.lay_p, self.lay_b, self.lay_c = layout
        self.drop_p = dropout_p if (train and variant == "unet") else 0.0
        self.drop_seed = drop_seed & 0xFFFFFFFF
        self.drop_salt = torch.zeros(1, dtype=torch.int32, device=device)
        self.head_off = head_offsets(self.heads)
        self.keep = []
        self.pack_ops, self.fwd_ops, self.bwd_ops = [], [], []
        self._pack_descs = []
        self._w_layout = {}
        self.recs = []
        self._ws_need = 0
        self._ws_users = []
        self._colsum_need = 0
        self._colsum_users = []
        self._build()
        Engine._live.add(self)

    def dropout_seed(self, nth_forward):
        return (self.drop_seed + nth_forward * DROP_STEP) & 0xFFFFFFFF

    def P(self, name):
        off, n = self.lay_p[name]
        return self.params.data_ptr() + 4 * off

    def G(self, name):
        off, n = self.lay_p[name]
        return self.grads.data_ptr() + 4 * off

    def Bf(self, name):
        off, n = self.lay_b[name]
        return self.buffers.data_ptr() + 4 * off

    def Cn(self, name):
        return self.counters.data_ptr() + 8 * self.lay_c[name]

    GUARD_BYTES = 4096

    def new(self, shape, dtype=None, fill=0.0):
        dtype = dtype or self.tdt
        if not self.guards:
            t = torch.full(shape, fill, dtype=dtype, device=self.dev)
            self.keep.append(t)
            return t
        n = 1
        for s_ in shape:
            n *= s_
        esz = torch.empty((), dtype=dtype).element_size()
        body = -(-n * esz // 256) * 256
        raw = torch.full((body + 2 * self.GUARD_BYTES,), 0xA5, dtype=torch.uint8, device=self.dev)
        t = raw[self.GUARD_BYTES:self.GUARD_BYTES + n * esz].view(dtype).view(shape)
        t.fill_(fill)
        self.keep.append(t)
        self._guarded.append((raw, n * esz, tuple(shape), str(dtype)))
        return t

    def check_guards(self):
        if not self.guards:
            raise RuntimeError("this plan was built without guards (Engine(guards=True) / Trainer(guards=True))")
        bad = []
        for i, (raw, nbytes, shape, dt) in enumerate(self._guarded):
            G = self.GUARD_BYTES
            lo_ok = bool((raw[:G] == 0xA5).all())
            hi_ok = bool((raw[G + nbytes:] == 0xA5).all())
            if not (lo_ok and hi_ok):
                bad.append((i, shape, dt, "below" if not lo_ok else "above"))
        if bad:
            raise RuntimeError("out-of-bounds stores next to %d of %d plan buffers: %s" % (len(bad), len(self._guarded), bad[:8]))
        return len(self._guarded)

    def act_buf(self, H, W, C, dt=None):
        t = self.new((self.B, H, W, C), self._tdt(dt)) if dt is not None else self.new((self.B, H, W, C))
        coef = (self.new((C,), torch.float32, 1.0), self.new((C,), torch.float32, 0.0), self.new((C,), torch.float32, 1.0))
        return t, coef

    def _emit(self, ops, fn, args, what, writes=(), meta=None):
        args = [C.byref(a) if isinstance(a, C.Structure) else a for a in args]
        ops.append(Op(fn, args, what, tuple(writes), meta or {"kernel": what.split(" ")[0], "flops": 0, "bytes": 0}))
        return args

    def _ew_meta(self, kernel, npix, Cn, passes, dt=None):
        return {"kernel": kernel, "flops": 0, "bytes": float(npix * Cn * self._esz(self.dt if dt is None else dt) * passes)}

    def _batch(self, descs, metas, kernel):
        arr = (type(descs[0]) * len(descs))(*descs)
        return arr, {"kernel": kernel, "flops": sum(m["flops"] for m in metas), "bytes": sum(m["bytes"] for m in metas)}

    def _flush_reduce(self, ops):
        pr = getattr(self, "_pending_reduce", None)
        if pr is not None:
            self._pending_reduce = None
            pops, rd, what, writes, meta = pr
            self._emit(pops, self.lib.abc_wgrad_reduce, (rd,), what, writes=writes, meta=meta)

    def _emit_bn_bwd(self, ops, f, what, writes):
        pr = getattr(self, "_pending_reduce", None)
        if pr is None or pr[0] is not ops or not self.merge_reduce:
            self._flush_reduce(ops)
            self._emit(ops, self.lib.abc_bn_finalize_bwd, (f,), what, writes=writes)
            return
        self._pending_reduce = None
        _pops, rd, rwhat, rwrites, rmeta = pr
        meta = {"ws": rmeta.get("ws", 0), "kernel": "wgrad_reduce+bn_bwd", "flops": 0, "bytes": rmeta["bytes"]}
        self._emit(ops, self.lib.abc_wgrad_reduce_bn_bwd, (rd, f), rwhat + " + " + what, tuple(rwrites) + tuple(writes), meta)

    def _dn(self, dt):
        return {L.BF16: "bf16", L.F32: "f32", L.FP8: "fp8"}[dt]

    def _esz(self, dt):
        return {L.BF16: 2, L.F32: 4, L.FP8: 1}[dt]

    def _tdt(self, dt):
        return {L.BF16: torch.bfloat16, L.F32: torch.float32, L.FP8: torch.float8_e4m3fn}[dt]

    FP8_OUT = ("up3.conv.double_conv.0", "up3.conv.double_conv.3", "dconv1.double_conv.0", "dconv1.double_conv.3",
               "dconv2.double_conv.0", "dconv2.double_conv.3")

    def _out_dt(self, cname):
        return L.FP8 if (self.fp8 and cname in self.FP8_OUT) else self.dt

    def emit_pack(self, wname, dst, mode, Cout, Cin, k, rows_pad, red_real, red_total=None, red_off=0, py=0, px=0, rows_total=0,
                  rows_off=0, row_scale=None, cdt=None):
        cdt = self.dt if cdt is None else cdt
        d = L.PackDesc()
        d.rows_total, d.rows_off = rows_total, rows_off
        d.row_scale = row_scale
        d.w, d.dst, d.mode, d.dtype_c = self.P(wname), dst.data_ptr(), mode, cdt
        d.Cout, d.Cin, d.kh, d.kw, d.py, d.px = Cout, Cin, k, k, py, px
        total = red_real if red_total is None else red_total
        ck = self.lib.abc_conv_chunk(cdt, total)
        d.rows_pad, d.red_pad, d.red_total, d.red_off, d.ck = rows_pad, -(-red_real // ck) * ck, total, red_off, ck
        self._pack_descs.append(d)

    def packed(self, ntaps, red, rows_pad, cdt=None):
        cdt = self.dt if cdt is None else cdt
        ck = self.lib.abc_conv_chunk(cdt, red)
        if ck <= 0:
            raise ValueError("no K-chunk for %d reduction channels in %s" % (red, self._dn(cdt)))
        return self.new((ntaps * (-(-red // ck)) * rows_pad * ck,), self._tdt(cdt))

    def _pack_weights(self, wname, mode, cout, cin, k):
        rows, red = (cout, cin) if mode == 0 else (cin, cout)
        rows_pad = -(-rows // 32) * 32
        w = self.packed(k * k, red, rows_pad)
        self.emit_pack(wname, w, mode, cout, cin, k, rows_pad, red)
        return w
# ... 461 lines not shown

    def _finish_build(self):
        lib = self.lib
        isz = lib.abc_pack_item_bytes()
        host = (C.c_char * (isz * len(self._pack_descs)))()
        first, elems = 0, 0
        for i, pd in enumerate(self._pack_descs):
            pd.layout = self._w_layout.get(pd.dst, 0)
            n = lib.abc_pack_item_fill(C.addressof(host) + i * isz, C.byref(pd), first)
            if n < 0:
                L.check(-1, "pack_item_fill")
            first += n
            ntaps = {0: pd.kh * pd.kw, 1: pd.kh * pd.kw, 2: (2 if pd.py else 1) * (2 if pd.px else 1), 3: 9}[pd.mode]
            elems += ntaps * pd.red_pad * pd.rows_pad
        table = torch.frombuffer(bytearray(bytes(host)), dtype=torch.uint8).to(self.dev)
        self.keep.append(table)
        self._emit(self.pack_ops, lib.abc_pack_batch, (table.data_ptr(), len(self._pack_descs), first), "pack weights",
                   meta={"kernel": "pack_batch", "flops": 0, "bytes": float(elems * (2 if self.dt == L.BF16 else 4) + elems * 4)})
        self.ws = [self.new((max(self._ws_need, 4),), torch.float32)]
        for d, k in self._ws_users:
            d.partial = self.ws[k].data_ptr()
        self.cs_ws = self.new((max(self._colsum_need, 4),), torch.float32)
        for a in self._colsum_users:
            a[7] = self.cs_ws.data_ptr()

    def _build_heads(self, trunk: Src):
        h, w = trunk.H, trunk.W
        nh = len(self.heads)
        self.h, self.w = h, w
        f8_feat = self.fp8 and trunk.dt == L.FP8 and trunk.C == 128 and nh <= 8 and self.batched_heads and (h * w) % 64 == 0
        self.hepi = None
        if self.fold and self.heads_epilogue and self.batched_heads and self.dt == L.BF16 and trunk.C == 128 and nh <= 8 and \
                (trunk.dt == L.BF16 or f8_feat):
            self.hepi = torch.zeros(nh * C.sizeof(L.HeadsEpi), dtype=torch.uint8, device=self.dev)
            self.keep.append(self.hepi)
        if self.hepi is not None:
            self.hfeat = self.new((1, 1, 1, 128 * nh), self._tdt(L.FP8) if f8_feat else None)
            self.hcoef = None
        else:
            self.hfeat, self.hcoef = self.act_buf(h, w, 128 * nh, L.FP8 if f8_feat else None)
        if f8_feat:
            self.hfeat_q = (self.new((nh,), torch.float32, 0.0), self.new((nh,), torch.float32, 1.0), self.new((nh,), torch.float32, 1.0))
        epi_items = []
        self.logits = [self.new((self.B, hc, h, w), torch.float32) for hc in self.heads]
        self.head_recs, self.head2 = [], []
        head_convs, head_fins = [], []
        self.hmean, self.hinvstd = self.new((128 * nh,), torch.float32), self.new((128 * nh,), torch.float32, 1.0)
        batch_fin = nh <= 8 and self.batched_heads
        shared = None
        if batch_fin and self.dt == L.BF16 and trunk.C == 128:
            shared = self._heads_conv1_merged(trunk, h, w)
        fused = self.want_fused_heads and shared is not None and (h * w) % 128 == 0 \
            and self.B * h * w * 128 * nh < (1 << 30)
        for i, hc in enumerate(self.heads):
            p = "out_modules.%d" % i
            rec, f = self.conv_bn(p + ".conv1", p + ".bn", trunk, 128, 3, (self.hfeat, self.hcoef, h, w, 128 * nh, 128 * i), 0.01,
                                  stat_out=(self.hmean[128 * i:128 * (i + 1)], self.hinvstd[128 * i:128 * (i + 1)]),
                                  collect_fin=head_fins if batch_fin else None, shared=shared)
            rec.is_head = True
            self.head_recs.append(rec)
            f.drop_p, f.drop_seed, f.drop_salt = self.drop_p, self.drop_seed, self.drop_salt
            if not fused:
                rows_pad = -(-hc // 32) * 32
                if self.hfeat_q is not None:
                    f.dt, f.q = L.FP8, tuple(t[i:i + 1] for t in self.hfeat_q)
                    qmul, deq = self._fp8_weight_scales(p + ".conv2.weight", hc, 128, None, f.q[1], self.new((hc,), torch.float32, 1.0),
                                                        self.new((hc,), torch.float32, 1.0))
                    w2 = self.packed(1, 128, rows_pad, cdt=L.FP8)
                    self.emit_pack(p + ".conv2.weight", w2, 0, hc, 128, 1, rows_pad, 128, row_scale=qmul.data_ptr(), cdt=L.FP8)
                    if self.hepi is not None:
                        epi_items.append((w2, self.P(p + ".conv2.bias"), deq, self.logits[i], hc, rows_pad))
                    else:
                        self.emit_conv(self.fwd_ops, f, w2, self.P(p + ".conv2.bias"), self.logits[i], L.F32, h, w, hc, 0, hc,
                                       [(0, 0)], what="fwd %s.conv2" % p, planar_out=True, collect=head_convs, cdt=L.FP8, out_scale=deq)
                    self.head2.append(Rec(kind="head2", cname=p + ".conv2", src=f, cout=hc, idx=i))
                    continue
                w2 = self._pack_weights(p + ".conv2.weight", 0, hc, 128, 1)
                if self.hepi is not None:
                    epi_items.append((w2, self.P(p + ".conv2.bias"), None, self.logits[i], hc, rows_pad))
                else:
                    self.emit_conv(self.fwd_ops, f, w2, self.P(p + ".conv2.bias"), self.logits[i], L.F32, h, w, hc, 0, hc,
                                   [(0, 0)], what="fwd %s.conv2" % p, planar_out=True, collect=head_convs)
            self.head2.append(Rec(kind="head2", cname=p + ".conv2", src=f, cout=hc, idx=i))
        if head_fins:
            arr = (L.BnFwdDesc * len(head_fins))(*head_fins)
            self._emit(self.fwd_ops, self.lib.abc_bn_finalize_fwd_batch, (arr, len(head_fins), 128 * nh if shared is not None else 0),
                       "bn out_modules.*.bn", meta={"kernel": "bn", "flops": 0, "bytes": 0})
        if fused:
            self._heads_fused_setup()
            return
        if self.hepi is not None:
            host = (L.HeadsEpi * nh)()
            for i, (w2, bias_ptr, deq, lg, hc, rows_pad) in enumerate(epi_items):
                host[i].w2, host[i].bias, host[i].oscale = w2.data_ptr(), bias_ptr, (None if deq is None else deq.data_ptr())
                host[i].y, host[i].Cout, host[i].Cout_pad = lg.data_ptr(), hc, rows_pad
            self.hepi.copy_(torch.frombuffer(bytearray(bytes(host)), dtype=torch.uint8))
            self.keep.append(epi_items)
            return
        if self.nms_heads and self.heads == arch.TRAIN_HEADS and len(head_convs) == 8:
            d6, d7 = head_convs[6][0], head_convs[7][0]
            rho, om = self.new((self.B, 60, h, w), torch.float32), self.new((self.B, 60, h, w), torch.float32)
            d6.head_aux, d6.head_aux_mode = rho.data_ptr(), 1
            d7.head_aux, d7.head_aux_mode = om.data_ptr(), 2
            if self.lib.abc_conv_variant(C.byref(d6)) == 3 and self.lib.abc_conv_variant(C.byref(d7)) == 3:
                self.nms_rho, self.nms_omega = rho, om
                head_convs[7][2]["bytes"] += float(self.B * 60 * h * w * 4)
                head_convs[6][2]["bytes"] += float(self.B * 60 * h * w * 4)
                if self.decode:
                    d5 = head_convs[5][0]
                    idx = self.new((self.B, 60, h, w), torch.uint8)
                    y5, y6 = d5.y, d6.y
                    d5.head_aux, d5.head_aux_mode, d5.y, d6.y = idx.data_ptr(), 3, None, None
                    if self.lib.abc_conv_variant(C.byref(d5)) == 3 and self.lib.abc_conv_variant(C.byref(d6)) == 3:
                        self.btype_idx = idx
                        head_convs[5][2]["bytes"] -= float(self.B * 360 * h * w * 4 - self.B * 60 * h * w)
                        head_convs[6][2]["bytes"] -= float(self.B * 60 * h * w * 4)
                        for dead in (self.logits[5], self.logits[6]):
                            self.keep[:] = [t for t in self.keep if t is not dead]
                        self.logits[5] = self.logits[6] = None
                    else:
                        d5.head_aux, d5.head_aux_mode, d5.y, d6.y = None, 0, y5, y6
                        self.decode = False
            else:
                d6.head_aux = d7.head_aux = None
                d6.head_aux_mode = d7.head_aux_mode = 0
        self.emit_heads_batch(self.fwd_ops, head_convs, 0, "fwd out_modules.*.conv2")

    def _heads_fused_setup(self):
        lib, nh, B, h, w = self.lib, len(self.heads), self.B, self.h, self.w
        Ct = 128 * nh
        d = L.HeadsFusedDesc()
        sc, sh, sl = self.hcoef
        d.feat, d.ld = self.hfeat.data_ptr(), Ct
        d.scale, d.shift, d.slope = sc.data_ptr(), sh.data_ptr(), sl.data_ptr()
        d.mean, d.invstd = self.hmean.data_ptr(), self.hinvstd.data_ptr()
        d.drop_p, d.drop_seed = self.drop_p, self.drop_seed
        d.drop_salt = self.drop_salt.data_ptr() if self.drop_p > 0 else None
        d.B, d.h, d.w = B, h, w
        nchunk = lib.abc_heads_fused_chunks(C.byref(d))
        self.hf_pack = self.new((lib.abc_heads_fused_pack_bytes() // 4 + 4,), torch.float32)
        self.hf_dl = self.new((lib.abc_heads_fused_dl_elems(C.byref(d)),), torch.bfloat16)
        self.hf_g = self.new((B, h, w, Ct))
        self.hf_bnpart = self.new((nchunk, 2, Ct), torch.float32)
        self.hf_lossblocks = lib.abc_heads_fused_loss_blocks(C.byref(d))
        self.hf_losspart = torch.zeros((self.hf_lossblocks, 16), dtype=torch.float64, device=self.dev)
        self.chan_scale = self.new((sum(self.heads),), torch.float32, 0.0)
        self.hf_work = self.new((lib.abc_heads_fused_wgrad_floats(C.byref(d)),), torch.float32)
        d.w2_pack, d.dl, d.g = self.hf_pack.data_ptr(), self.hf_dl.data_ptr(), self.hf_g.data_ptr()
        d.bn_partial, d.loss_partial = self.hf_bnpart.data_ptr(), self.hf_losspart.data_ptr()
        d.chan_scale, d.wgrad_work = self.chan_scale.data_ptr(), self.hf_work.data_ptr()
        if self.drop_p > 0:
            self.hf_keep = self.new((3 * B * h * w * 16,), torch.uint8, 0)
            d.keep_mask = self.hf_keep.data_ptr()
        for i in range(nh):
            p = "out_modules.%d.conv2" % i
            d.w2[i], d.b2[i], d.logits[i] = self.P(p + ".weight"), self.P(p + ".bias"), self.logits[i].data_ptr()
            d.dw2[i], d.db2[i], d.chan_off[i] = self.G(p + ".weight"), self.G(p + ".bias"), self.head_off[i]
        self.hf, self.hf_chunks = d, nchunk
        self._emit(self.pack_ops, lib.abc_heads_fused_pack, (d,), "pack out_modules.*.conv2", meta={"kernel": "heads_fused_pack", "flops": 0, "bytes": 0})

    def _heads_conv1_merged(self, trunk: Src, h, w):
        nh = len(self.heads)
        Ct = 128 * nh
        taps = taps_square(3)
        wf = self.packed(len(taps), 128, Ct)
        bias_all = self.new((Ct,), torch.float32)
        if self.fold:
            scale_all = self.new((Ct,), torch.float32, 1.0)
            f8 = trunk.dt == L.FP8
            if f8:
                wf = self.packed(len(taps), 128, Ct, cdt=L.FP8)
                qmul_all, deq_all = self.new((Ct,), torch.float32, 1.0), self.new((Ct,), torch.float32, 1.0)
            for i in range(nh):
                p = "out_modules.%d" % i
                sl = slice(128 * i, 128 * (i + 1))
                self._fold_coeffs(p + ".conv1", p + ".bn", 128, scale_all[sl], bias_all[sl])
                if f8:
                    self._fp8_weight_scales(p + ".conv1.weight", 128, 128 * 9, scale_all[sl], trunk.q[1], qmul_all[sl], deq_all[sl])
                    self.emit_pack(p + ".conv1.weight", wf, 0, 128, 128, 3, 128, 128, rows_total=Ct, rows_off=128 * i,
                                   row_scale=qmul_all[sl].data_ptr(), cdt=L.FP8)
                else:
                    self.emit_pack(p + ".conv1.weight", wf, 0, 128, 128, 3, 128, 128, rows_total=Ct, rows_off=128 * i,
                                   row_scale=scale_all[sl].data_ptr())
            self.emit_conv(self.fwd_ops, trunk, wf, bias_all.data_ptr(), self.hfeat, L.FP8 if self.hfeat_q is not None else self.dt, h, w, Ct, 0, Ct, taps,
                           what="fwd out_modules.*.conv1", out_slope=0.01, cdt=L.FP8 if f8 else None, out_scale=deq_all if f8 else None,
                           out_quant=None if self.hfeat_q is None else self.hfeat_q[2], out_quant_stride=0 if self.hfeat_q is None else 1,
                           heads_epi=self.hepi)
            return None, 0
        for i in range(nh):
            self.emit_pack("out_modules.%d.conv1.weight" % i, wf, 0, 128, 128, 3, 128, 128, rows_total=Ct, rows_off=128 * i)
        srcs = (C.c_void_p * nh)(*[self.P("out_modules.%d.conv1.bias" % i) for i in range(nh)])
        counts = (C.c_int32 * nh)(*([128] * nh))
        bp = bias_all.data_ptr()
        self._emit(self.pack_ops, self.lib.abc_concat_f32, (srcs, counts, nh, bp), "gather out_modules.*.conv1.bias",
                   meta={"kernel": "concat", "flops": 0, "bytes": 0})
        return self.emit_conv(self.fwd_ops, trunk, wf, bp, self.hfeat, self.dt, h, w, Ct, 0, Ct, taps, stats=self.train,
                              what="fwd out_modules.*.conv1")

    def _act_bwd(self, ops, rec, same, pool, g_ptr, ld_g, drop=None):
        C_ = rec.cout
        d = L.ActBwdDesc()
        d.y_raw, d.ld_y = rec.y.data_ptr(), rec.ld
        if same is not None:
            d.dA_same, d.ld_same, d.csame_off = same[0].data_ptr(), same[1], same[2]
        if pool is not None:
            d.dA_pool, d.ld_pool, d.cpool_off = pool[0].data_ptr(), pool[1], pool[2]
        d.g, d.ld_g = g_ptr, ld_g
        d.scale, d.shift, d.slope = rec.scale.data_ptr(), rec.shift.data_ptr(), rec.slopes.data_ptr()
        d.mean, d.invstd = rec.mean.data_ptr(), rec.invstd.data_ptr()
        d.dtype, d.B, d.H, d.W, d.C, d.cy_off = self.dt, self.B, rec.H, rec.W, C_, rec.coff
        if drop is not None:
            d.drop_p, d.drop_seed, d.drop_ld, d.drop_salt = drop[0], drop[1], rec.ld, self.drop_salt.data_ptr()
        nblk = self.lib.abc_act_bwd_blocks(C.byref(d))
        part = self.new((nblk, 2, C_), torch.float32)
        d.partial = part.data_ptr()
        nsrc = (1 if d.dA_same else 0) + (0.25 if d.dA_pool else 0)
        self._emit(ops, self.lib.abc_act_bwd, (d,), "act_bwd " + rec.bname, meta=self._ew_meta("act_bwd", self.B * rec.H * rec.W, C_, 2 + nsrc))
        return part, nblk

    def _bn_bwd_desc(self, rec, part_ptr, nblk, coefs=None, in_scale=None):
        C_ = rec.cout
        k = tuple(self.new((C_,), torch.float32) for _ in range(3))
        f = L.BnBwdDesc()
        f.partial, f.nblk, f.C, f.count = part_ptr, nblk, C_, float(self.B * rec.H * rec.W)
        f.gamma, f.invstd = self.P(rec.bname + ".weight"), rec.invstd.data_ptr()
        f.dgamma, f.dbeta = self.G(rec.bname + ".weight"), self.G(rec.bname + ".bias")
        f.k1, f.k2, f.gscale = (t.data_ptr() for t in k)
        if coefs is not None:
            f.mean = rec.mean.data_ptr()
            f.ca, f.cb, f.cc = (t.data_ptr() for t in coefs)
        f.in_scale = in_scale
        return f, k, (rec.bname + ".weight", rec.bname + ".bias")

    def _bn_backward(self, ops, rec, same=None, pool=None, drop=None, defer=False, g=None, partials=None, in_place=False):
        C_ = rec.cout
        fg = getattr(rec, "fused_g", None)
        if fg is not None:
            assert pool is None and drop is None
            g, partials = (fg[0], C_, 0), fg[1:]
        if g is None:
            g = (self.new((self.B, rec.H, rec.W, C_)), C_, 0)
            rec.g = g[0]
        gt, ld_g, g_off = g
        g_ptr = gt.data_ptr() + g_off * gt.element_size()
        part, nblk = partials or self._act_bwd(ops, rec, same, pool, g_ptr, ld_g, drop)
        coefs = tuple(self.new((C_,), torch.float32) for _ in range(3)) if defer else None
        f, (k1, k2, gs), writes = self._bn_bwd_desc(rec, part.data_ptr(), nblk, coefs)
        self._emit_bn_bwd(ops, f, "bn_bwd " + rec.bname, writes)
        a = L.BnApplyDesc()
        a.g, a.ld_g, a.y_raw, a.ld_y, a.cy_off = g_ptr, ld_g, rec.y.data_ptr(), rec.ld, rec.coff
        a.mean, a.invstd, a.k1, a.k2, a.gscale = rec.mean.data_ptr(), rec.invstd.data_ptr(), k1.data_ptr(), k2.data_ptr(), gs.data_ptr()
        a.dtype, a.C, a.npix = self.dt, C_, self.B * rec.H * rec.W

        def emit_apply():
            out = g
            if not in_place:
                out = (self.new((self.B, rec.H, rec.W, C_)), C_, 0)
                a.out, a.ld_out = out[0].data_ptr(), C_
            self._emit(ops, self.lib.abc_bn_apply_bwd, (a,), "bn_apply " + rec.bname, meta=self._ew_meta("bn_apply", self.B * rec.H * rec.W, C_, 3))
            if out[1] == C_:
                rec.dY = out[0]
            return Src(out[0], self.dt, rec.H, rec.W, out[1], out[2], C_)

        if defer:
            assert g_off == 0
            ca, cb, cc = coefs
            return Src(gt, self.dt, rec.H, rec.W, ld_g, 0, C_, coef=(ca, cc, cb)), emit_apply
        return emit_apply()

    def _conv_backward(self, ops, rec, dY, want_dgrad=True, into=None):
        if isinstance(dY, tuple) and not self.dual_wgrad:
            dY = dY[1]()
        if isinstance(dY, tuple):
            gsrc, emit_apply = dY
            out = self.new((self.B, rec.H, rec.W, rec.cout))
            if self.emit_wgrad(ops, gsrc, rec.src, rec.cout, rec.cin, rec.taps, 1, rec.cname + ".weight", "wgrad " + rec.cname,
                               dual=(rec.y, rec.ld, rec.coff, out.data_ptr(), rec.cout)):
                rec.dY = out
                dY = Src(out, self.dt, rec.H, rec.W, rec.cout, 0, rec.cout)
            else:
                dY = emit_apply()
                self.emit_wgrad(ops, dY, rec.src, rec.cout, rec.cin, rec.taps, 1, rec.cname + ".weight", "wgrad " + rec.cname)
        else:
            self.emit_wgrad(ops, dY, rec.src, rec.cout, rec.cin, rec.taps, 1, rec.cname + ".weight", "wgrad " + rec.cname)
        prod = rec.src.producer
        if not want_dgrad or prod is None:
            return None
        lh, lw = rec.src.lh()
        wd = self._pack_weights(rec.cname + ".weight", 1, rec.cout, rec.cin, rec.k)
        rec.dsrc_accumulated = False
        if into is not None and self.dt == L.BF16 and tuple(into.shape) == (self.B, lh, lw, rec.cin):
            got = self.emit_conv(ops, dY, wd, None, into, self.dt, lh, lw, rec.cin, 0, rec.cin, taps_mirror(rec.taps),
                                 what="dgrad " + rec.cname + " (+= d(out) of the identity residual)", accumulate=True, only_variant=5)
            if got is not None:
                rec.dsrc, rec.dsrc_accumulated = into, True
                return into
        dsrc = self.new((self.B, lh, lw, rec.cin))
        rec.dsrc = dsrc
        tgt = self._actbwd_target(rec)
        if tgt is not None:
            got = self.emit_conv(ops, dY, wd, None, dsrc, self.dt, lh, lw, rec.cin, 0, rec.cin, taps_mirror(rec.taps),
                                 what="dgrad " + rec.cname + " + act_bwd " + tgt.bname, actbwd=tgt)
            if got is not None:
                tgt.fused_g = (dsrc, got[0], got[1])
                tgt.g = dsrc
                rec.dsrc_is_g = True
# ... 399 lines not shown
```

abc-net_amd/model.py:

```python
from __future__ import annotations

import ctypes as C
import threading
import weakref
from collections import OrderedDict

import torch
import torch.nn as nn

from . import _lib as L
from . import arch
from .engine import Engine


GRAD_STORE_ALIGN = 840 * 128


def _kaiming_uniform_(t, fan_in, gen=None):
    b = 1.0 / (fan_in ** 0.5)
    with torch.no_grad():
        t.uniform_(-b, b, generator=gen)


class _UNetFn(torch.autograd.Function):
# ... 50 lines not shown
    holds the reference-named parameters and buffers, which are views into the model's flat arenas"""


class UNetBase(nn.Module):
    VARIANT = "unet"

    def __init__(self, in_channels, heads=None, dtype="fp32", dropout_p=0.2):
        super().__init__()
        heads = list(arch.DEFAULT_HEADS if heads is None else heads)
        self.n_channels = in_channels
        self.heads = heads
        self.compute_dtype = dtype
        self.dropout_p = dropout_p
        self.dropout_seed_base = 0x1234ABCD
        self.dropout_seed = self.dropout_seed_base
        self._table = arch.state_table(self.VARIANT, in_channels, heads)
        self._lay_p, self._np = arch.arena_layout(self._table, "param")
        self._lay_b, self._nb = arch.arena_layout(self._table, "buffer")
        self._lay_c = OrderedDict((n, i) for i, (n, s, r) in enumerate(t for t in self._table if t[2] == "counter"))
        self._flat = torch.zeros(self._np)
        self._flat_buf = torch.zeros(self._nb)
        self._counters = torch.zeros(len(self._lay_c), dtype=torch.int64)
        self._flat_grad = None
        self._grad_store = None
        self._engines = {}
        self._master_ref = weakref.ref(self)
        self._dp_shadows = {}
        self._dp_lock = threading.Lock()
        self._dp_busy = False
        self._leaves = []
        self._param_slices = []
        for name, shape, role in self._table:
            *path, attr = name.split(".")
            mod = self
            for seg in path:
                nxt = mod._modules.get(seg)
                if nxt is None:
                    nxt = _Node()
                    mod.add_module(seg, nxt)
                mod = nxt
            v = self._view(name)
            if role == "param":
                mod.register_parameter(attr, nn.Parameter(v))
                off, cnt = self._lay_p[name]
                self._param_slices.append((off, cnt, tuple(shape)))
            else:
                mod.register_buffer(attr, v)
            self._leaves.append((name, mod, attr, role))
        self.reset_parameters()

    def __reduce__(self):
        return (_rebuild_unet, (type(self), self.n_channels, list(self.heads), self.compute_dtype, self.dropout_p,
                                self._flat.detach().cpu().clone(), self._flat_buf.detach().cpu().clone(), self._counters.cpu().clone(),
                                str(self._flat.device), self.training, self.dropout_seed_base,
                                [p.requires_grad for p in self.parameters()]))

    def __deepcopy__(self, memo):
        fn, args = self.__reduce__()
        new = fn(*args)
        memo[id(self)] = new
        return new

    def _shape_role(self, name):
        for n, shape, role in self._table:
            if n == name:
                return shape, role
        raise KeyError(name)

    def _view(self, name):
        shape, role = self._shape_role(name)
        if role == "param":
            off, cnt = self._lay_p[name]
            return self._flat[off:off + cnt].view(shape)
        if role == "buffer":
            off, cnt = self._lay_b[name]
            return self._flat_buf[off:off + cnt].view(shape)
        return self._counters[self._lay_c[name]]

    def _rebind(self):
        for name, mod, attr, role in self._leaves:
            v = self._view(name)
            if role == "param":
                p = mod._parameters[attr]
                p.data = v
                p.grad = None
            else:
                mod._buffers[attr] = v

    def _apply(self, fn, recurse=True):
        flat, buf = fn(self._flat), fn(self._flat_buf)
        cnt = fn(self._counters)
        if flat.dtype != torch.float32 or buf.dtype != torch.float32 or cnt.dtype != torch.int64:
            raise L.AbcNetHipError("abcnet_amd keeps its parameters in float32 (the compute dtype is the constructor's dtype=)")
        moved = flat.device != self._flat.device
        self._flat, self._flat_buf, self._counters = flat, buf, cnt
        if moved:
            self._flat_grad = None
            self._engines = {}
        self._rebind()
        return self

    def reset_parameters(self, seed=None):
        gen = None
        if seed is not None:
            gen = torch.Generator().manual_seed(seed)
        fan = {}
        for name, shape, role in self._table:
            if role == "param" and name.endswith(".weight") and len(shape) >= 2:
                f = shape[1]
                for d in shape[2:]:
                    f *= d
                fan[name[:-7]] = f
        with torch.no_grad():
            for name, shape, role in self._table:
                v = self._view(name)
                if v.device.type != "cpu":
                    raise L.AbcNetHipError("reset_parameters(): initialise on the host, then .to(device)")
                if role == "param":
                    if name == "s":
                        v.copy_(torch.randn(10, generator=gen) / 100)
                    elif len(shape) >= 2:
                        _kaiming_uniform_(v, fan[name[:-7]], gen)
                    elif name.endswith(".bias") and name[:-5] in fan:
                        _kaiming_uniform_(v, fan[name[:-5]], gen)
                    elif name.endswith(".weight"):
                        v.fill_(1.0)
                    else:
                        v.zero_()
                elif role == "buffer":
                    v.fill_(1.0 if name.endswith("running_var") else 0.0)
                else:
                    v.zero_()

    def named_reference_parameters(self):
        for name, shape, role in self._table:
            if role == "param":
                yield name, self._view(name)

    def grad_of(self, name):
        off, cnt = self._lay_p[name]
        return self._flat_grad[off:off + cnt].view(self._shape_role(name)[0])

    def flat_param_grads(self):
        return torch.cat([(p.grad if p.grad is not None else torch.zeros_like(p)).reshape(-1) for p in self.parameters()])

    def load_state_dict(self, state_dict, strict=True, assign=False):
        if assign:
            raise L.AbcNetHipError("load_state_dict(assign=True) would detach the parameters from the arena")
        if state_dict and all(k.startswith("module.") for k in state_dict.keys()):
            state_dict = OrderedDict((k[7:], v) for k, v in state_dict.items())
        return super().load_state_dict(state_dict, strict=strict)

    def _engine_for(self, x, train, fold_bn=False, fused_heads=False, batched_heads=True, fp8=False, guards=False, heads_epilogue=False,
                    actbwd_epilogue=True, merge_reduce=True, nms_heads=False, decode=False, dual_wgrad=True, fused_convt=True):
        if not x.is_cuda:
            raise L.AbcNetHipError("abcnet_amd runs on an MI355X only (got a %s tensor); there is no CPU fallback" % x.device)
        if x.device != self._flat.device:
            raise L.AbcNetHipError("input on %s but the model lives on %s (move one of them; several GPUs: nn.DataParallel(model, "
                                   "device_ids=...) or, better, one process per GPU -- abcnet_amd.distributed.launch_ranks / torchrun)"
                                   % (x.device, self._flat.device))
        B, Cc, H, W = x.shape
        if Cc != self.n_channels:
            raise ValueError("expected %d input channels, got %d" % (self.n_channels, Cc))
        key = (B, H, W, bool(train), self.compute_dtype, self.dropout_seed, bool(fold_bn), bool(fused_heads), bool(batched_heads), bool(fp8), bool(guards), bool(heads_epilogue), bool(actbwd_epilogue), bool(merge_reduce),
               bool(nms_heads), bool(decode), bool(dual_wgrad), bool(fused_convt), L.load().abc_get_reserved_cus())
        eng = self._engines.get(key)
        if eng is None or eng.params.data_ptr() != self._flat.data_ptr():
            if self._flat_grad is None or self._flat_grad.device != x.device:
                pad = -(-self._np // GRAD_STORE_ALIGN) * GRAD_STORE_ALIGN
                self._grad_store = torch.zeros(pad, dtype=torch.float32, device=x.device)
                self._flat_grad = self._grad_store[:self._np]
            with torch.cuda.device(x.device):
                eng = Engine(self.VARIANT, self.n_channels, self.heads, self._flat, self._flat_grad, self._flat_buf,
                             self._counters, (self._lay_p, self._lay_b, self._lay_c), B, H, W, self.compute_dtype, train,
                             dropout_p=self.dropout_p, device=x.device, drop_seed=self.dropout_seed, fold_bn=fold_bn,
                             fused_heads=fused_heads, batched_heads=batched_heads, fp8=fp8, guards=guards, heads_epilogue=heads_epilogue, nms_heads=nms_heads,
                             actbwd_epilogue=actbwd_epilogue, merge_reduce=merge_reduce, decode=decode, dual_wgrad=dual_wgrad, fused_convt=fused_convt)
            self._engines[key] = eng
        return eng

    def _load_image(self, eng, x):
        eng.img.copy_(x.reshape(eng.img.shape))

    def _export_logits(self, eng, st):
        return [t.clone() for t in eng.logits]

    def _replica_tensors(self):
        params, bufs, cnts = [], [], []
        for name, shape, role in self._table:
            *path, attr = name.split(".")
            mod = self
            for seg in path:
                mod = mod._modules[seg]
            if role == "param":
                params.append(mod._former_parameters[attr])
            elif role == "buffer":
                bufs.append(mod._buffers[attr])
            else:
                cnts.append(mod._buffers[attr])
        return params, bufs, cnts

    def _dp_release(self, token=None):
        lock = getattr(self, "_dp_lock", None)
        if lock is None:
            self._dp_busy = False
            return
        with lock:
            if token is None or getattr(self, "_dp_token", None) is token:
                self._dp_busy = False
                self._dp_token = None

    def _dp_checkout(self, master, dev):
        with master._dp_lock:
            if dev == master._flat.device and not master._dp_busy:
                master._dp_busy = True
                return master
            pool = master._dp_shadows.setdefault(dev, [])
            for sh in pool:
                if not sh._dp_busy:
                    sh._dp_busy = True
                    return sh
            if len(pool) >= 4:
                raise L.AbcNetHipError("nn.DataParallel: more than 4 unfinished forward passes on %s (a training forward holds its "
                                       "engine until its backward has run)" % dev)
            fn, args = master.__reduce__()
            args = list(args)
            args[8] = str(dev)
            sh = fn(*args)
            sh._dp_busy = True
            pool.append(sh)
            return sh

    def _forward_replica(self, x):
        master = self._master_ref()
        if master is None:
            raise L.AbcNetHipError("nn.DataParallel replica without its master module")
        dev = x.device
        params, bufs, cnts = self._replica_tensors()
        owner = self._dp_checkout(master, dev)
        try:
            if owner is not master:
                with torch.no_grad():
                    torch.cat([p.detach().reshape(-1) for p in params], out=owner._flat)
                    torch.cat([b.reshape(-1).to(torch.float32) for b in bufs], out=owner._flat_buf)
                    owner._counters.copy_(torch.stack([c.reshape(()) for c in cnts]))
                from .distributed import rank_dropout_seed
                owner.dropout_seed = rank_dropout_seed(master.dropout_seed_base, 1 + (dev.index or 0) + 16 * master._dp_shadows[dev].index(owner))
            owner.train(self.training)
            with torch.cuda.device(dev):
                if torch.is_grad_enabled() and self.training:
                    outs = list(_UNetFn.apply(owner, x, *params))
                    token = owner._dp_token = object()
                    node = outs[0].grad_fn
                    if node is not None:
                        weakref.finalize(node, owner._dp_release, token)
                    else:
                        owner._dp_release()
                    return outs
                eng = owner._engine_for(x, self.training)
                st = torch.cuda.current_stream().cuda_stream
                owner._load_image(eng, x)
                eng.run_pack(st)
                eng.run_forward(st)
                outs = owner._export_logits(eng, st)
            owner._dp_release()
            return list(outs)
        except Exception:
            owner._dp_release()
            raise

    def forward(self, x):
        if getattr(self, "_is_replica", False):
            return self._forward_replica(x)
        if torch.is_grad_enabled() and self.training:
            outs = _UNetFn.apply(self, x, *self.parameters())
        else:
            eng = self._engine_for(x, self.training)
            with torch.cuda.device(x.device):
                st = torch.cuda.current_stream().cuda_stream
                self._load_image(eng, x)
                eng.run_pack(st)
                eng.run_forward(st)
                outs = self._export_logits(eng, st)
        return list(outs)

    def forward_logits(self, x):
        eng = self._engine_for(x, self.training)
        with torch.cuda.device(x.device):
            st = torch.cuda.current_stream().cuda_stream
            self._load_image(eng, x)
            eng.run_pack(st)
            eng.run_forward(st)
        return eng.logits, eng

    def nms(self, x):
        from .ops import check_nms_heads, nms_peaks
        check_nms_heads(self.heads, "model.nms")
        lg, eng = self.forward_logits(x)
        return nms_peaks(lg[0], lg[4], lg[6], lg[7])
```

abc-net_amd/train.py:

```python
from __future__ import annotations

import os

import torch

from . import _lib as L
from . import distributed as D
from .contract import HEADS, alloc_targets, check_sparse_rasterizer, current_stream, refuse_dense_targets, resolve_device
from .ops import FusedAdam, FusedHeadsLoss, FusedLoss, FusedMetrics, fold_marks, meters_dict, per_iteration, timed


class Trainer:
    def __init__(self, model, batch, height, width, lr=2.5e-4, weight_decay=1e-8, use_graph=True, bucket_mb=8.0,
                 process_group=None, device=None, metrics=False, broadcast_buffers="lazy", fused_heads=True, keep_logits=True,
                 batched_heads=True, exchange="all_reduce", force_exchange=False, guards=False, actbwd_epilogue=True, merge_reduce=True,
                 reserve_cus=None, dual_wgrad=True, fused_convt=True, exchange_dtype="f32"):
        if exchange_dtype not in D.GradReducer.WIRE_DTYPES:
            raise ValueError("Trainer: exchange_dtype must be one of %s, got %r" % (D.GradReducer.WIRE_DTYPES, exchange_dtype))
        if exchange_dtype == "bf16" and exchange != "direct":
            raise ValueError("Trainer: exchange_dtype='bf16' needs exchange='direct' (the local f32 sum between all-to-all and "
                             "all-gather), got exchange=%r" % (exchange,))
        if tuple(model.heads) != HEADS:
            raise ValueError("Trainer: the fused training step is defined for heads %s (train.py:47), got heads %s"
                             % (list(HEADS), list(model.heads)))
        self.dev = dev = resolve_device(model, device, "Trainer")
        self.model = model
        dist_on = torch.distributed.is_initialized()
        self.world = torch.distributed.get_world_size(process_group) if dist_on else 1
        self.rank = torch.distributed.get_rank(process_group) if dist_on else 0
        self.group = process_group
        if broadcast_buffers not in ("step", "lazy", False):
            raise ValueError("broadcast_buffers must be 'step', 'lazy' or False")
        self.broadcast_buffers = broadcast_buffers if self.world > 1 else False
        model.dropout_seed = D.rank_dropout_seed(model.dropout_seed_base, self.rank)
        model.train()
        from .engine import set_reserved_cus
        self.reserve_cus = L.load().abc_get_reserved_cus() if reserve_cus is None else set_reserved_cus(reserve_cus)
        with torch.cuda.device(dev):
            x0 = torch.zeros((batch, model.n_channels, height, width), device=dev)
            self.eng = model._engine_for(x0, True, fused_heads=fused_heads, batched_heads=batched_heads, guards=guards,
                                         actbwd_epilogue=actbwd_epilogue, merge_reduce=merge_reduce, dual_wgrad=dual_wgrad, fused_convt=fused_convt)
        eng = self.eng
        self.targets = alloc_targets(batch, eng.h, eng.w, dev)
        off_s, _ = model._lay_p["s"]
        extra = {"keep_logits": bool(keep_logits or metrics)} if eng.hf is not None else {}
        self.loss = (FusedHeadsLoss if eng.hf is not None else FusedLoss)(
            eng, self.targets, model._flat.data.data_ptr() + 4 * off_s, model._flat_grad.data_ptr() + 4 * off_s, grad_scale=1.0 / self.world, **extra)
        self.metrics = FusedMetrics(eng.logits, self.targets) if metrics else None
        self.lr, self.wd = lr, weight_decay
        self.opt = FusedAdam(model._flat.data, model._flat_grad, lr=lr, weight_decay=weight_decay)
        names = list(model._lay_p.keys())
        sizes = [model._lay_p[n][1] for n in names]
        ready = {n: -1 for n in names}
        for j, (_fn, _args, _what, writes, _meta) in enumerate(eng.bwd_ops):
            for n in writes:
                ready[n] = max(ready[n], j)
        rd = [ready[n] for n in names]
        self.buckets = D.plan_buckets(rd, sizes, int(bucket_mb * (1 << 20) / 4))
        store = getattr(model, "_grad_store", None)
        align = 128 * self.world
        self.exchange_on = self.world > 1 or (bool(force_exchange) and dist_on)
        if self.exchange_on and exchange != "all_reduce" and store is not None and store.numel() % align == 0 \
                and store.data_ptr() == model._flat_grad.data_ptr():
            self.buckets = D.align_buckets(self.buckets, sizes, rd, align, store.numel())
            self.reducer = D.GradReducer(store, self.buckets, process_group, mode=exchange, force=force_exchange, wire_dtype=exchange_dtype)
        else:
            self.reducer = D.GradReducer(model._flat_grad, self.buckets, process_group, mode="all_reduce", force=force_exchange)
            if self.exchange_on and exchange_dtype == "bf16":
                self.reducer.fallback_reason = "the gradient store does not split into buckets of 128 x world elements: f32 all_reduce instead of the bf16 exchange"
        self.use_graph = use_graph
        self._graphs = None
        self._segments = self._plan_segments()
        self.steps = 0
        self._buffers_synced_at = 0
        self._loss_acc = torch.zeros(2, dtype=torch.float64, device=dev)

    def load_batch(self, imgs, targets=None):
        self.eng.img.copy_(imgs.reshape(self.eng.img.shape), non_blocking=True)
        if targets is None:
            return
        refuse_dense_targets(getattr(self, "_rasterizer", None))
        for dst, src in zip(self.targets, targets):
            dst.copy_(src, non_blocking=True)

    @property
    def input_images(self):
        return self.eng.img

    def use_sparse_targets(self, rasterizer):
        if not hasattr(self.loss, "use_target_flags"):
            raise L.AbcNetHipError("sparse targets need the fused heads pass (bf16, fused_heads=True)")
        if rasterizer is None:
            self.loss.use_target_flags(None)
            self._rasterizer = None
        else:
            check_sparse_rasterizer(rasterizer, self.targets, "Trainer")
            self.loss.use_target_flags(rasterizer.group_flags)
            self._rasterizer = rasterizer
        self._graphs = None

    def reset_optimizer(self, lr):
        self.lr = lr
        self.opt = FusedAdam(self.model._flat.data, self.model._flat_grad, lr=lr, weight_decay=self.wd)
        self._graphs = None

    def _plan_segments(self):
        eng = self.eng
        pre = [eng.run_pack, eng.run_forward, self.loss.run]
        if self.metrics is not None:
            pre.append(self.metrics.run)
        cut = sorted(set(b[2] for b in self.buckets)) if self.exchange_on else []
        segs, seg_b = [], []
        cur = list(pre)
        start = 0
        ops = eng.bwd_ops
        early = [b for b in self.buckets if b[2] < 0]
        for c in [c for c in cut if c >= 0]:
            chunk = ops[start:c + 1]
            cur.append(lambda st, chunk=chunk: eng._run(chunk, st))
            segs.append(cur)
            seg_b.append([b for b in self.buckets if b[2] == c])
            cur = []
            start = c + 1
        tail = ops[start:]
        if tail:
            cur.append(lambda st, chunk=tail: eng._run(chunk, st))
        segs.append(cur)
        seg_b.append([])
        self._early = early
        self._seg_buckets = seg_b
        return segs

    def _run_segment(self, k):
        st = current_stream(self.dev)
        for fn in self._segments[k]:
            fn(st)

    def _capture(self):
        graphs = []
        for k in range(len(self._segments)):
            if not self._segments[k]:
                graphs.append(None)
                continue
            g = torch.cuda.CUDAGraph()
            with torch.cuda.graph(g, capture_error_mode="thread_local"):
                self._run_segment(k)
            graphs.append(g)
        gopt = torch.cuda.CUDAGraph()
        with torch.cuda.graph(gopt, capture_error_mode="thread_local"):
            self.opt.step()
        self._graphs = (graphs, gopt)

    def sync_buffers(self):
        if self.world > 1:
            with torch.cuda.device(self.dev):
                D.broadcast_buffers(self.model._flat_buf, self.model._counters, group=self.group)
        self._buffers_synced_at = self.steps

    def accumulate_loss(self):
        self._loss_acc[0] += self.loss.total_device()
        self._loss_acc[1] += 1

    def read_loss_mean(self, reset=True):
        acc = self._loss_acc.clone()
        if self.world > 1:
            torch.distributed.all_reduce(acc, op=torch.distributed.ReduceOp.SUM, group=self.group)
        s, n = acc.tolist()
        if reset:
            self._loss_acc.zero_()
        return s / max(n, 1.0)

    def step(self):
        with torch.cuda.device(self.dev):
            if self.broadcast_buffers == "step":
                D.broadcast_buffers(self.model._flat_buf, self.model._counters, group=self.group)
            self._step()

    def _step(self):
        if self.use_graph and self._graphs is None and self.steps >= 1:
            torch.cuda.synchronize()
            self._capture()
        graphs = self._graphs
        for k in range(len(self._segments)):
            if graphs is not None:
                if graphs[0][k] is not None:
                    graphs[0][k].replay()
            else:
                self._run_segment(k)
            if k == 0:
                for lo, hi, _ in self._early:
                    self.reducer.bucket_ready(lo, hi)
            for lo, hi, _ in self._seg_buckets[k]:
                self.reducer.bucket_ready(lo, hi)
        self.reducer.finish()
# ... 92 lines not shown
```

include/abcnet_hip.h:

```cpp
#ifndef ABCNET_HIP_H
#define ABCNET_HIP_H
#include <stdint.h>

#ifdef __cplusplus
extern "C" {
#endif

typedef void* abc_stream_t;

enum abc_status { ABC_OK = 0, ABC_EINVAL = -1, ABC_EUNSUPPORTED = -2, ABC_ELAUNCH = -3 };
enum abc_dtype { ABC_F32 = 0, ABC_BF16 = 1, ABC_FP8 = 2  };
#define ABC_MAX_TAPS_C 49

typedef struct abc_act_src {
    const void* x;
    const float* scale;
    const float* shift;
    const float* slope;
    int32_t Hx, Wx, ldx;
    int32_t pool;
    float drop_p;
    uint32_t drop_seed;
    int32_t planar;
    int32_t ctot;
// ... 101 lines not shown
int abc_bn_eval_fold(const float* gamma, const float* beta, const float* running_mean, const float* running_var,
                     const float* conv_bias, float* scale, float* bias_out, int32_t C, float eps, abc_stream_t stream);

typedef struct abc_act_bwd_desc {
    const void* y_raw; int32_t ld_y;
    const void* dA_same; int32_t ld_same;
    const void* dA_pool; int32_t ld_pool;
    void* g; int32_t ld_g;
    float* partial;
    const float* scale; const float* shift; const float* slope; const float* mean; const float* invstd;
    int32_t dtype, B, H, W, C, cy_off, csame_off, cpool_off;
    float drop_p; uint32_t drop_seed; int32_t drop_ld;
    const uint32_t* drop_salt;
} abc_act_bwd_desc;
int abc_act_bwd_blocks(const abc_act_bwd_desc* d);
int abc_act_bwd(const abc_act_bwd_desc* d, abc_stream_t stream);
typedef struct abc_bn_bwd_desc {
    const float* partial; int32_t nblk; int32_t C; double count;
    const float* gamma; const float* invstd;
    float* dgamma; float* dbeta; float* k1; float* k2; float* gscale;
    const float* mean; float* ca; float* cb; float* cc;
    const float* in_scale;
} abc_bn_bwd_desc;
int abc_bn_finalize_bwd(const abc_bn_bwd_desc* d, abc_stream_t stream);
int abc_bn_finalize_bwd_batch(const abc_bn_bwd_desc* descs, int32_t n, int32_t pstride, abc_stream_t stream);
typedef struct abc_bn_apply_desc {
    void* g; int32_t ld_g; const void* y_raw; int32_t ld_y; int32_t cy_off;
    const float* mean; const float* invstd; const float* k1; const float* k2; const float* gscale;
    int32_t dtype, C; int64_t npix;
    void* out; int32_t ld_out;
} abc_bn_apply_desc;
int abc_bn_apply_bwd(const abc_bn_apply_desc* d, abc_stream_t stream);

typedef struct abc_wgrad_desc {
    abc_act_src p;
    abc_act_src q;
    float* partial;
    int32_t dtype_p, dtype_q, dtype_c;
    int32_t B, Hg, Wg;
    int32_t Hq, Wq;
    int32_t cp_off, Ca, cq_off, Cb;
    int32_t stride, ntaps, nsplit;
    int8_t tap_dy[ABC_MAX_TAPS_C];
    int8_t tap_dx[ABC_MAX_TAPS_C];
    const void* p2; int32_t ld_p2, cp2_off, p_dual; void* p_out; int32_t ld_pout;
    float* rowsum_partial;
} abc_wgrad_desc;
int abc_wgrad_rowsum_ok(const abc_wgrad_desc* d);
int abc_wgrad_fuses_apply(const abc_wgrad_desc* d);
int abc_wgrad_pads(const abc_wgrad_desc* d, int32_t* ca_pad, int32_t* cb_pad);
int abc_wgrad_tile(const abc_wgrad_desc* d, int32_t* at, int32_t* bt);
int abc_wgrad_route_info(const abc_wgrad_desc* d, int32_t* info);
int abc_wgrad_blocks(const abc_wgrad_desc* d);
int abc_wgrad(const abc_wgrad_desc* d, abc_stream_t stream);
typedef struct abc_wgrad_reduce_desc {
    const float* partial; int32_t nsplit, ntaps, Ca, Cb, Ca_pad, Cb_pad;
    float* dw;
    int32_t accumulate;
} abc_wgrad_reduce_desc;
int abc_wgrad_heads_batch(const abc_wgrad_desc* descs, int32_t n, abc_stream_t stream);
int abc_wgrad_reduce(const abc_wgrad_reduce_desc* d, abc_stream_t stream);
int abc_wgrad_reduce_bn_bwd(const abc_wgrad_reduce_desc* r, const abc_bn_bwd_desc* f, abc_stream_t stream);
int abc_wgrad_reduce_batch(const abc_wgrad_reduce_desc* descs, int32_t n, abc_stream_t stream);

int abc_colsum_blocks(int64_t npix);
int abc_colsum(const void* x, int32_t dtype, int64_t npix, int32_t ld, int32_t c_off, int32_t C,
               const float* chan_scale, float* work , float* out, abc_stream_t stream);
int abc_colsum_w1(const void* x, int32_t dtype, int64_t npix, int32_t ld, int32_t c_off, int32_t C, const float* w,
                  float* work, float* out_sum, float* out_w, abc_stream_t stream);

typedef struct abc_loss_desc {
    const float* logits[8]; float* dlogits[8];
    const float* t_atom; const float* t_types; const float* t_charges; const float* t_hs; const float* t_bond;
    const float* t_btypes; const double* t_rho; const double* t_omega;
    int32_t B, h, w;
    double* partial;
} abc_loss_desc;
int abc_loss_blocks(const abc_loss_desc* d);
int abc_loss_fwd_bwd(const abc_loss_desc* d, abc_stream_t stream);
typedef struct abc_loss_fin_desc {
    const double* partial; int32_t nblk;
    const float* s; float* ds;
    double* out;
    float* chan_scale; int32_t nchan;
    int32_t chan_off[8]; int32_t head_c[8];
    float grad_scale;
} abc_loss_fin_desc;
int abc_loss_finalize(const abc_loss_fin_desc* d, abc_stream_t stream);
typedef struct abc_loss_scale_desc {
    float* dlogits[8]; int64_t n[8];
    const float* head_scale;
    float* ds;
    const double* grad_out;
} abc_loss_scale_desc;
int abc_loss_scale_grads(const abc_loss_scale_desc* d, abc_stream_t stream);

int abc_plane_sum_work(int32_t C);
int abc_plane_sum(const float* x, int32_t B, int32_t C, int32_t HW, const float* chan_scale, float* work, float* out,
                  abc_stream_t stream);

typedef struct abc_adam_desc {
    float* p; const float* g; float* m; float* v; int64_t n;
    int64_t* step;
    float lr, beta1, beta2, eps, weight_decay, grad_scale;
} abc_adam_desc;
int abc_adam_step(const abc_adam_desc* d, abc_stream_t stream);

#define ABC_ADAM_MAX_CLASSES 32
typedef struct abc_adam_seg {
    float* p; const float* g; float* m; float* v;
    int64_t n;
    int64_t first_chunk;
    int32_t cls;
    int32_t pad_;
} abc_adam_seg;
typedef struct abc_adam_class {
    float step_size;
    float bc2_sqrt;
    float beta1, beta2, eps, weight_decay;
    float pad_[2];
} abc_adam_class;
typedef struct abc_adam_multi_desc {
    const abc_adam_seg* segs;
    int32_t nseg;
    int32_t nclass;
    int64_t chunk_total;
    abc_adam_class cls[ABC_ADAM_MAX_CLASSES];
} abc_adam_multi_desc;
int abc_adam_multi_chunk(void);
int abc_adam_multi(const abc_adam_multi_desc* d, abc_stream_t stream);

int abc_heads_batch(const abc_conv_desc* descs, int32_t n, int32_t which, abc_stream_t stream);

typedef struct abc_heads_fused_desc {
    const void* feat; int32_t ld;
    const float* scale; const float* shift; const float* slope;
    const float* mean; const float* invstd;
    float drop_p; uint32_t drop_seed; const uint32_t* drop_salt;
    const float* w2[8]; const float* b2[8];
    void* w2_pack;
    float* logits[8];
    const float* t_atom; const float* t_types; const float* t_charges; const float* t_hs; const float* t_bond;
    const float* t_btypes; const double* t_rho; const double* t_omega;
    void* dl;
    void* g;
    float* bn_partial;
    double* loss_partial;
    int32_t B, h, w;
    const float* chan_scale; int32_t chan_off[8];
    float* dw2[8]; float* db2[8];
    float* wgrad_work;
    void* keep_mask;
    const uint32_t* target_flags; const void* zero_bytes;
} abc_heads_fused_desc;
int64_t abc_heads_fused_pack_bytes(void);
int abc_heads_fused_chunks(const abc_heads_fused_desc* d);
int abc_heads_fused_loss_blocks(const abc_heads_fused_desc* d);
int64_t abc_heads_fused_dl_elems(const abc_heads_fused_desc* d);
int64_t abc_heads_fused_wgrad_floats(const abc_heads_fused_desc* d);
int abc_heads_fused_rows(int32_t head);
int abc_heads_fused_chan_of_row(int32_t head, int32_t row);
int abc_heads_fused_pack(const abc_heads_fused_desc* d, abc_stream_t stream);
int abc_heads_fused_fwd_bwd(const abc_heads_fused_desc* d, abc_stream_t stream);
int abc_heads_fused_wgrad(const abc_heads_fused_desc* d, abc_stream_t stream);

typedef struct abc_nms_desc {
    const float* atom; const float* bond; const float* rho; const float* omega;
    int32_t B, h, w, n_omega;
    float* atom_mask; float* bond_mask; float* rho_abs; float* omega_mask;
} abc_nms_desc;
int abc_nms_peaks(const abc_nms_desc* d, abc_stream_t stream);

typedef struct abc_raster_desc {
    float* t_atom; float* t_types; float* t_charges; float* t_hs; float* t_bond; float* t_btypes; double* t_rho; double* t_omega;
    int32_t B, h, w, max_atoms, max_bonds;
    const int32_t* atoms; const int32_t* n_atoms;
    const int32_t* bonds; const int32_t* n_bonds;
    const double* rho;
    uint32_t* group_flags;
    int32_t* prev_atoms; int32_t* prev_bonds; double* prev_rho; int32_t* prev_counts;
    int32_t incremental;
} abc_raster_desc;
int abc_rasterize_targets(const abc_raster_desc* d, abc_stream_t stream);

enum abc_image_param { ABC_IMG_SRC_H = 0, ABC_IMG_SRC_W, ABC_IMG_ROWS, ABC_IMG_COLS, ABC_IMG_DDX, ABC_IMG_DDY, ABC_IMG_SALT_THR,
                       ABC_IMG_PEPPER_THR, ABC_IMG_KEY_LO, ABC_IMG_KEY_HI, ABC_IMG_NPARAM };
enum abc_image_mode { ABC_IMG_TRAIN = 0, ABC_IMG_TEST = 1 };
typedef struct abc_image_desc {
    float* out;
    const uint8_t* src;
    int64_t src_stride;
    int32_t src_pitch;
    int32_t src_max_h;
    const int32_t* params;
    const int32_t* params_host;
    int32_t B, S, mode;
    int32_t test_max_ink;
} abc_image_desc;
int abc_build_images(const abc_image_desc* d, abc_stream_t stream);

enum abc_scan_param { ABC_SCAN_SRC_H = 0, ABC_SCAN_SRC_W, ABC_SCAN_NPARAM };
enum abc_scan_polarity { ABC_SCAN_DARK = 0, ABC_SCAN_LIGHT = 1, ABC_SCAN_AUTO = 2 };
enum abc_scan_status { ABC_SCAN_CONSTANT = 1, ABC_SCAN_BAD_PARAMS = 2 };
enum abc_scan_geom { ABC_SCAN_G_THR = 0, ABC_SCAN_G_INVERTED, ABC_SCAN_G_STATUS, ABC_SCAN_G_Y0, ABC_SCAN_G_X0, ABC_SCAN_G_BH,
                     ABC_SCAN_G_BW, ABC_SCAN_G_ROWS, ABC_SCAN_G_COLS, ABC_SCAN_G_DDX, ABC_SCAN_G_DDY, ABC_SCAN_G_INK, ABC_SCAN_NGEOM };
enum { ABC_SCAN_NBOX = 8 };
typedef struct abc_scan_desc {
    float* out;
    const uint8_t* src;
    int64_t src_stride;
    int32_t src_pitch;
    int32_t src_max_h;
    const int32_t* params;
    const int32_t* params_host;
    int32_t B, S;
    int32_t margin;
    int32_t cover_q8;
    int32_t polarity;
    uint32_t* hist;
    int32_t* box;
    int32_t* geom;
} abc_scan_desc;
int abc_build_scan_images(const abc_scan_desc* d, abc_stream_t stream);
int abc_scan_desc_size(void);

enum abc_scan_clean_status { ABC_SCAN_NO_COMPONENT = 4, ABC_SCAN_CLEAN_FAILED = 8 };
enum abc_scan_clean_stat { ABC_SCAN_C_COMPONENTS = 0, ABC_SCAN_C_KEPT, ABC_SCAN_C_INK_KEPT, ABC_SCAN_C_INK_DROPPED,
                           ABC_SCAN_C_HEAVIEST, ABC_SCAN_C_OCCUPIED, ABC_SCAN_NCLEAN };
typedef struct abc_scan_clean_desc {
    void* scratch;
    int32_t* stats;
    int32_t* labels_out;
    uint8_t* keep_out;
    int32_t cell;
    int32_t min_ink;
    int32_t keep_q8;
} abc_scan_clean_desc;
int abc_build_scan_images_clean(const abc_scan_desc* d, const abc_scan_clean_desc* q, abc_stream_t stream);
int abc_scan_clean_desc_size(void);
int64_t abc_scan_clean_scratch_bytes(int32_t B, int32_t src_max_h, int32_t src_pitch, int32_t cell);

enum { ABC_STROKE_UNTIL_STABLE = -1, ABC_STROKE_MAX_SIZE = 1024 };
enum abc_stroke_stat { ABC_STROKE_ITERATIONS = 0, ABC_STROKE_CONVERGED, ABC_STROKE_INK_IN, ABC_STROKE_INK_OUT, ABC_STROKE_SKIPPED,
                       ABC_STROKE_NSTAT };
typedef struct abc_stroke_desc {
    const float* src;
    float* dst;
    int32_t B, S;
    int32_t drop_isolated;
    int32_t max_iter;
    int32_t radius;
    int32_t skip_stride;
    const int32_t* skip;
    int32_t* stats;
} abc_stroke_desc;
int abc_normalize_strokes(const abc_stroke_desc* d, abc_stream_t stream);
int abc_stroke_desc_size(void);

enum abc_decoder_limit { ABC_MAX_CAP_ATOMS = 2048, ABC_MAX_BOND_PEAKS = 4096, ABC_MAX_SCORE_RECORD = 1024, ABC_MAX_SIM_ATOMS = 512 };

enum abc_omega_rule { ABC_OMEGA_RAW = 0, ABC_OMEGA_PEAKS = 1 };
typedef struct abc_extract_desc {
    const float* atom_mask; const float* bond_mask;
    const float* types; const float* charges; const float* hs;
    const float* btypes; const float* rho; const float* omega;
    int32_t B, h, w, cap_atoms, cap_bonds;
    int32_t* counts;
    int32_t* atoms;
    int32_t* bonds;
    float* bond_rho;
    int32_t* work;
    uint64_t* work_masks;
    const uint8_t* btype_idx;
    int32_t omega_rule;
} abc_extract_desc;
int64_t abc_extract_work_ints(const abc_extract_desc* d);
int64_t abc_extract_work_masks(const abc_extract_desc* d);
int abc_extract_peaks(const abc_extract_desc* d, abc_stream_t stream);

enum abc_mol_status { ABC_MOL_EMPTY = 1, ABC_MOL_TRUNCATED = 2 };
enum abc_text_status { ABC_TEXT_BAD_ROW = 4, ABC_TEXT_OVERFLOW = 8 };
typedef struct abc_assemble_desc {
    const int32_t* counts;
    const int32_t* atoms;
    const int32_t* bonds;
    const float* bond_rho;
    const double* trig;
    int32_t B, cap_atoms, cap_bonds, cap_mol_bonds;
    int32_t* mol_counts;
    int32_t* mol_atoms;
    int32_t* mol_bonds;
    int32_t* mol_implh;
    int32_t* work;
} abc_assemble_desc;
int64_t abc_assemble_work_ints(const abc_assemble_desc* d);
int abc_assemble_graphs(const abc_assemble_desc* d, abc_stream_t stream);

typedef struct abc_metrics_desc {
    const float* logits[8];
    const float* t_atom; const float* t_types; const float* t_charges; const float* t_hs; const float* t_bond;
    const float* t_btypes; const double* t_rho; const double* t_omega;
    int32_t B, h, w;
    uint8_t* peaks;
    double* partial;
    double* totals;
    double* last;
// ... 174 lines not shown
```

Before: 2879 images/sec.

## Skip zero-target tiles in fused heads loss and downstream wgrad

Adds a per-wavefront ballot over the target maps so softmax heads whose targets are all zero for a pixel chunk take the existing skip path, and per-tile masks for head 5 that omit the logit GEMM, focal loss, dgrad MFMA and d(logits) stores for all-zero tiles. A 64-bit tile mask per chunk is written and consumed by the heads wgrad kernel to skip loading and computing on those d(logits) tiles. The aim is to cut work in the sparse-target heads, at the cost of extra ballots, branches and mask plumbing. Correctness depends on the skipped tiles truly contributing zero gradient, and a no_zero_skip flag keeps the old behaviour.

```diff
diff --git a/abc-net_amd/_lib.py b/abc-net_amd/_lib.py
--- a/abc-net_amd/_lib.py
+++ b/abc-net_amd/_lib.py
@@ -168,7 +168,8 @@
                 ("logits", vp * 8), ("t_atom", vp), ("t_types", vp), ("t_charges", vp), ("t_hs", vp), ("t_bond", vp),
                 ("t_btypes", vp), ("t_rho", vp), ("t_omega", vp), ("dl", vp), ("g", vp), ("bn_partial", vp), ("loss_partial", vp),
                 ("B", i32), ("h", i32), ("w", i32), ("chan_scale", vp), ("chan_off", i32 * 8), ("dw2", vp * 8), ("db2", vp * 8),
-                ("wgrad_work", vp), ("keep_mask", vp), ("target_flags", vp), ("zero_bytes", vp)]
+                ("wgrad_work", vp), ("keep_mask", vp), ("target_flags", vp), ("zero_bytes", vp),
+                ("dl_tiles", vp), ("no_zero_skip", i32), ("pad_", i32)]
 
 
 class ConvTDesc(C.Structure):
diff --git a/abc-net_amd/csrc/heads_fused.hip b/abc-net_amd/csrc/heads_fused.hip
--- a/abc-net_amd/csrc/heads_fused.hip
+++ b/abc-net_amd/csrc/heads_fused.hip
@@ -28,6 +28,8 @@
     const double *t_rho, *t_omega;
     const uint32_t* tflags;
     const char* tzero;
+    uint64_t* dl_tiles;
+    int noskip;
     float* bnpart;
     float* dwsmall;
     double* losspart;
@@ -42,7 +44,8 @@
 constexpr int WV = 16384;
 constexpr int LDS_BSUM = 4 * WV;
 constexpr int LDS_LSUM = LDS_BSUM + 4 * 2 * 2 * 128 * 4;
-constexpr int HF_LDS = LDS_LSUM + 4 * 16 * 8;
+constexpr int LDS_TMASK = LDS_LSUM + 4 * 16 * 8;
+constexpr int HF_LDS = LDS_TMASK + 16;
 
 struct Ctx {
     int lane, r, h, wave, chunk, b, yx, nslice;
@@ -52,6 +55,7 @@
     float* wsum;
     float dscale;
     uint32_t dseed;
+    uint32_t tmask;
 };
 
 typedef __attribute__((address_space(3))) bf16x4 lds_bf16x4_f;
@@ -105,6 +109,30 @@
         }
     }
     __syncthreads();
+}
+
+template <int HEAD>
+__device__ inline void zero_tail(const HFK& a, Ctx& c, uint32_t kb0, uint32_t kb1, double* lsum) {
+    const int slice = 128 * HEAD, lane = c.lane;
+    const u32x4 z4 = {0u, 0u, 0u, 0u};
+    const int sg = lane & 7, pg = lane >> 3;
+#pragma unroll
+    for (int half = 0; half < 2; ++half)
+#pragma unroll
+        for (int it = 0; it < 4; ++it)
+            *(u32x4*)(a.g + (size_t)(c.pix0 + it * 8 + pg) * a.ld + slice + 64 * half + sg * 8) = z4;
+    float* ws = c.wsum + c.nslice * 256;
+#pragma unroll
+    for (int i = 0; i < 4; ++i) ws[lane + 64 * i] = 0.f;
+    if constexpr (HEAD >= 5) {
+        if (a.hd[HEAD].keep != nullptr) a.hd[HEAD].keep[2u * c.pix + c.h] = make_uint2(kb0, kb1);
+    }
+    c.nslice += 1;
+    if (lane == 0) {
+        lsum[HEAD] = 0.0;
+        lsum[8 + HEAD] = 0.0;
+        if (HEAD == 5) lsum[8 + 6] = 0.0;
+    }
 }
 
 template <int HEAD>
@@ -190,13 +218,16 @@
             }
         }
     }
+    if constexpr (HEAD == 5) c.tmask = a.noskip ? 0x7FFFu : 0u;
+    if (HEAD != 5 || a.dl_tiles == nullptr || a.noskip) {
 #pragma unroll 1
-    for (int mt = 0; mt < NT; ++mt)
-#pragma unroll
-        for (int j = 0; j < 2; ++j) {
-            const int q = lane + 64 * j, row = q >> 2, part = q & 3;
-            *(u32x4*)((char*)(hd.dlb + ((size_t)c.chunk * CPAD + 32 * mt) * 128) + (uint32_t)((row * 128 + 32 * c.wave + part * 8) * 2)) = z4;
-        }
+        for (int mt = 0; mt < NT; ++mt)
+#pragma unroll
+            for (int j = 0; j < 2; ++j) {
+                const int q = lane + 64 * j, row = q >> 2, part = q & 3;
+                *(u32x4*)((char*)(hd.dlb + ((size_t)c.chunk * CPAD + 32 * mt) * 128) + (uint32_t)((row * 128 + 32 * c.wave + part * 8) * 2)) = z4;
+            }
+    }
     if constexpr (HEAD == 5) {
 #pragma unroll
         for (int j = 0; j < 30; ++j) c.dnl[j * 64 + lane] = 0.f;
@@ -209,26 +240,7 @@
         lds_sync();
         small_head_wgrad<HEAD>(a, c, fb);
     }
-    {
-        const int sg = lane & 7, pg = lane >> 3;
-#pragma unroll
-        for (int half = 0; half < 2; ++half)
-#pragma unroll
-            for (int it = 0; it < 4; ++it)
-                *(u32x4*)(a.g + (size_t)(c.pix0 + it * 8 + pg) * a.ld + slice + 64 * half + sg * 8) = z4;
-        float* ws = c.wsum + c.nslice * 256;
-#pragma unroll
-        for (int i = 0; i < 4; ++i) ws[lane + 64 * i] = 0.f;
-    }
-    if constexpr (HEAD >= 5) {
-        if (hd.keep != nullptr) hd.keep[2u * c.pix + h] = make_uint2(kbits[0], kbits[1]);
-    }
-    c.nslice += 1;
-    if (lane == 0) {
-        lsum[HEAD] = 0.0;
-        lsum[8 + HEAD] = 0.0;
-        if (HEAD == 5) lsum[8 + 6] = 0.0;
-    }
+    zero_tail<HEAD>(a, c, kbits[0], kbits[1], lsum);
 }
 
 template <int HEAD>
@@ -256,6 +268,16 @@
     float* bl = (float*)(c.ot + WV_BIAS);
     const uint32_t e0 = c.pix * (uint32_t)a.ld + slice + 8 * h;
 
+    if constexpr (HEAD == 1 || HEAD == 2 || HEAD == 3) {
+        if (!a.noskip) {
+            const float* tg = HEAD == 1 ? a.t_types : (HEAD == 2 ? a.t_charges : a.t_hs);
+            bool nz = false;
+#pragma unroll
+            for (int k = 0; k < CH; ++k) nz |= *at4(tg, k) != 0.f;
+            if (__builtin_amdgcn_ballot_w64(nz) == 0) { run_head_skip<HEAD>(a, c, lsum); return; }
+        }
+    }
+
     u32x4 raw[8];
 #pragma unroll
     for (int kk = 0; kk < 8; ++kk) raw[kk] = *(const u32x4*)(a.y1 + e0 + 16 * kk);
@@ -337,10 +359,20 @@
             for (int mi = 0; mi < 4; ++mi) accD[mi] = __builtin_amdgcn_mfma_f32_32x32x16_bf16(wt[4 * u + mi], bqp[u], accD[mi], 0, 0, 0);
     };
 
+    uint32_t tmask = 0u;
+    bool prev = false;
 #pragma unroll 1
     for (int mt = 0; mt < NT; ++mt) {
-        if (PIPE && mt > 0) dgrad_mfma();
+        if (PIPE && mt > 0 && prev) dgrad_mfma();
         if constexpr (!PIPE) load_fa(mt);
+        bool fired = true;
+        if constexpr (HEAD == 5) {
+            bool nz = false;
+#pragma unroll
+            for (int k = 0; k < 12; ++k) nz |= tn[k] != 0.f;
+            fired = a.noskip != 0 || __builtin_amdgcn_ballot_w64(nz) != 0;
+            tmask |= (fired ? 1u : 0u) << mt;
+        }
         f32x16 acc;
 #pragma unroll
         for (int q = 0; q < 4; ++q) {
@@ -348,32 +380,41 @@
 #pragma unroll
             for (int j = 0; j < 4; ++j) acc[4 * q + j] = b4[j];
         }
-#pragma unroll
-        for (int kk = 0; kk < 8; ++kk) acc = __builtin_amdgcn_mfma_f32_32x32x16_bf16(fa[kk], fb[kk], acc, 0, 0, 0);
+        if (fired || st_logits) {
+#pragma unroll
+            for (int kk = 0; kk < 8; ++kk) acc = __builtin_amdgcn_mfma_f32_32x32x16_bf16(fa[kk], fb[kk], acc, 0, 0, 0);
+        }
         float v[16], dlv[16];
 #pragma unroll
         for (int k = 0; k < 16; ++k) { v[k] = acc[k]; dlv[k] = 0.f; }
         if constexpr (HEAD == 5) {
-#pragma unroll
-            for (int gi = 0; gi < 2; ++gi) {
-                float z[6], t[6], dz[6], dn = 0.f;
-#pragma unroll
-                for (int k = 0; k < 6; ++k) { z[k] = v[8 * gi + k]; t[k] = tn[6 * gi + k]; }
-                num += (double)class_focal<6, true>(z, t, nullptr, dz, &dn);
-                den += (double)dn;
-                c.dnl[(2 * mt + gi) * 64 + lane] = dn;
-#pragma unroll
-                for (int k = 0; k < 6; ++k) dlv[8 * gi + k] = dz[k];
+            if (fired) {
+#pragma unroll
+                for (int gi = 0; gi < 2; ++gi) {
+                    float z[6], t[6], dz[6], dn = 0.f;
+#pragma unroll
+                    for (int k = 0; k < 6; ++k) { z[k] = v[8 * gi + k]; t[k] = tn[6 * gi + k]; }
+                    num += (double)class_focal<6, true>(z, t, nullptr, dz, &dn);
+                    den += (double)dn;
+                    c.dnl[(2 * mt + gi) * 64 + lane] = dn;
+#pragma unroll
+                    for (int k = 0; k < 6; ++k) dlv[8 * gi + k] = dz[k];
+                }
+            } else {
+                c.dnl[(2 * mt) * 64 + lane] = 0.f;
+                c.dnl[(2 * mt + 1) * 64 + lane] = 0.f;
             }
             __builtin_amdgcn_sched_barrier(0);
             {
                 const int mtn = mt + 1 < NT ? mt + 1 : mt;
                 load_fa(mtn);
-#pragma unroll
-                for (int u = 0; u < 2; ++u)
-#pragma unroll
-                    for (int mi = 0; mi < 4; ++mi)
-                        wt[4 * u + mi] = *(const bf16x8*)((const char*)(hd.w2t + (size_t)((2 * mt + u) * 128 + 32 * mi) * 16) + (uint32_t)(r * 32 + h * 16));
+                if (fired) {
+#pragma unroll
+                    for (int u = 0; u < 2; ++u)
+#pragma unroll
+                        for (int mi = 0; mi < 4; ++mi)
+                            wt[4 * u + mi] = *(const bf16x8*)((const char*)(hd.w2t + (size_t)((2 * mt + u) * 128 + 32 * mi) * 16) + (uint32_t)(r * 32 + h * 16));
+                }
                 load_t5(mtn);
             }
             __builtin_amdgcn_sched_barrier(0);
@@ -437,19 +478,29 @@
             }
         }
 
-        bqp[0] = pack_frag<bf16>(dlv);
-        bqp[1] = pack_frag<bf16>(dlv + 8);
-        char* tl = c.ot;
-#pragma unroll
-        for (int k = 0; k < 16; ++k) *(bf16*)(tl + ((k & 3) + 8 * (k >> 2) + 4 * h) * TROW + r * 2) = bqp[k >> 3][k & 7];
-        lds_sync();
-#pragma unroll
-        for (int j = 0; j < 2; ++j) {
-            const int q = lane + 64 * j, row = q >> 2, part = q & 3;
-            const u32x4 t = *(const u32x4*)(tl + row * TROW + part * 16);
-            *(u32x4*)((char*)(hd.dlb + ((size_t)c.chunk * CPAD + 32 * mt) * 128) + (uint32_t)((row * 128 + 32 * c.wave + part * 8) * 2)) = t;
-        }
-        lds_sync();
+        if (fired) {
+            bqp[0] = pack_frag<bf16>(dlv);
+            bqp[1] = pack_frag<bf16>(dlv + 8);
+            char* tl = c.ot;
+#pragma unroll
+            for (int k = 0; k < 16; ++k) *(bf16*)(tl + ((k & 3) + 8 * (k >> 2) + 4 * h) * TROW + r * 2) = bqp[k >> 3][k & 7];
+            lds_sync();
+#pragma unroll
+            for (int j = 0; j < 2; ++j) {
+                const int q = lane + 64 * j, row = q >> 2, part = q & 3;
+                const u32x4 t = *(const u32x4*)(tl + row * TROW + part * 16);
+                *(u32x4*)((char*)(hd.dlb + ((size_t)c.chunk * CPAD + 32 * mt) * 128) + (uint32_t)((row * 128 + 32 * c.wave + part * 8) * 2)) = t;
+            }
+            lds_sync();
+        } else if (a.dl_tiles == nullptr) {
+            const u32x4 z4 = {0u, 0u, 0u, 0u};
+#pragma unroll
+            for (int j = 0; j < 2; ++j) {
+                const int q = lane + 64 * j, row = q >> 2, part = q & 3;
+                *(u32x4*)((char*)(hd.dlb + ((size_t)c.chunk * CPAD + 32 * mt) * 128) + (uint32_t)((row * 128 + 32 * c.wave + part * 8) * 2)) = z4;
+            }
+        }
+        prev = fired;
         if constexpr (!PIPE) {
 #pragma unroll
             for (int u = 0; u < 2; ++u)
@@ -459,9 +510,13 @@
             if (mt + 1 < NT) dgrad_mfma();
         }
     }
+    if constexpr (HEAD == 5) {
+        c.tmask = tmask;
+        if (tmask == 0u) { zero_tail<HEAD>(a, c, kbits[0], kbits[1], lsum); return; }
+    }
 #pragma unroll
     for (int kk = 0; kk < 8; ++kk) raw[kk] = *(const u32x4*)(a.y1 + e0 + 16 * kk);
-    dgrad_mfma();
+    if (!PIPE || prev) dgrad_mfma();
 
     if constexpr (HEAD < 5) small_head_wgrad<HEAD>(a, c, fb);
 
@@ -554,6 +609,7 @@
     const int group = blockIdx.y;
     c.wsum = (float*)(smem + LDS_BSUM) + c.wave * 512;
     c.nslice = 0;
+    c.tmask = 0u;
     c.dscale = a.drop_p > 0.f ? 1.0f / (1.0f - a.drop_p) : 1.0f;
     c.dseed = a.drop_seed + ((a.drop_p > 0.f && a.drop_salt) ? *a.drop_salt : 0u);
     double* ls = (double*)(smem + LDS_LSUM);
@@ -569,7 +625,19 @@
         case 5: run_head<3>(a, c, lsum); break;
         default: run_head<4>(a, c, lsum); break;
     }
+    uint32_t* tm = (uint32_t*)(smem + LDS_TMASK);
+    if (group == 0 && c.lane == 0) tm[c.wave] = c.tmask;
     __syncthreads();
+    if (group == 0 && a.dl_tiles != nullptr && threadIdx.x == 0) {
+        uint64_t word = 0;
+#pragma unroll
+        for (int w = 0; w < 4; ++w) {
+            const uint32_t m = tm[w];
+#pragma unroll
+            for (int mt = 0; mt < 15; ++mt) word |= (uint64_t)((m >> mt) & 1u) << (4 * mt + w);
+        }
+        a.dl_tiles[c.chunk] = word;
+    }
     if (threadIdx.x < 16) {
         const int i = threadIdx.x & 7;
         const bool mine = group == 0 ? (i == 5 || i == 6) : (group == 1 ? i == 7 : i == group - 2);
@@ -660,6 +728,7 @@
     k.t_btypes = d->t_btypes; k.t_rho = d->t_rho; k.t_omega = d->t_omega;
     if ((d->target_flags != nullptr) != (d->zero_bytes != nullptr)) return abc_fail(ABC_EINVAL, "heads_fused: target_flags and zero_bytes go together");
     k.tflags = d->target_flags; k.tzero = (const char*)d->zero_bytes;
+    k.dl_tiles = d->dl_tiles; k.noskip = d->no_zero_skip != 0;
     k.bnpart = d->bn_partial; k.losspart = d->loss_partial; k.dwsmall = d->wgrad_work;
     k.HW = d->h * d->w; k.nchunk = abc_heads_fused_chunks(d);
     size_t row0 = 0;
diff --git a/abc-net_amd/csrc/wgrad_heads.hip b/abc-net_amd/csrc/wgrad_heads.hip
--- a/abc-net_amd/csrc/wgrad_heads.hip
+++ b/abc-net_amd/csrc/wgrad_heads.hip
@@ -18,6 +18,7 @@
     unsigned bytesP, bytesQ;
     int cpad_blk;
     const uint8_t* keep;
+    const uint64_t* tiles;
 };
 
 constexpr int HQ_PSW = 320;
@@ -61,8 +62,13 @@
     const __amdgpu_buffer_rsrc_t rsK = abc_make_rsrc(kmask ? a.keep : (const uint8_t*)a.q, kmask ? (unsigned)a.nchunks * 2048u : 0u);
     const unsigned kbyte = (unsigned)((part & 1) * 8 + (part >> 1));
     const int CPI = a.HW / 128;
-    auto issue = [&](int c, u32x4 (&qreg)[4], u32x4 (&preg)[8]) {
-        const bool live = c < c1;
+    auto tmask16 = [&](int c) -> uint32_t {
+        if (!BLK || a.tiles == nullptr) return 0xFFFFu;
+        if (c >= c1) return 0u;
+        return (uint32_t)__builtin_amdgcn_readfirstlane((int)(uint32_t)(a.tiles[c] >> (16 * mg))) & 0xFFFFu;
+    };
+    auto issue = [&](int c, const uint32_t m16, u32x4 (&qreg)[4], u32x4 (&preg)[8]) {
+        const bool live = c < c1 && m16 != 0u;
         const int b = c / CPI, pp0 = (c - b * CPI) * 128;
         const unsigned qoff = live ? (unsigned)(((unsigned)(c * 128 + pix0) * (unsigned)a.ldq + (unsigned)(a.cq_off + part * 8)) * 2u) : 0x80000000u;
 #pragma unroll
@@ -76,7 +82,8 @@
 #pragma unroll
             for (int i = 0; i < 4; ++i) {
                 const int row = mg * 128 + (tid >> 4) + 32 * i;
-                const unsigned poff = (live && row < a.cpad_blk) ? (unsigned)((((unsigned)c * (unsigned)a.cpad_blk + (unsigned)row) * 128u + 8u * (tid & 15)) * 2u) : 0x80000000u;
+                const bool bit = (m16 >> (4 * i + ((tid & 15) >> 2))) & 1u;
+                const unsigned poff = (live && bit && row < a.cpad_blk) ? (unsigned)((((unsigned)c * (unsigned)a.cpad_blk + (unsigned)row) * 128u + 8u * (tid & 15)) * 2u) : 0x80000000u;
                 preg[i] = __builtin_amdgcn_raw_buffer_load_b128(rsP, poff, 0, 0);
             }
         } else {
@@ -169,21 +176,24 @@
     constexpr int BUF = HEAD_PBUF + HEAD_QBUF;
     char* const b0 = smem;
     char* const b1 = smem + BUF;
-    issue(c0, qreg0, preg0);
-    issue(c0 + 1, qreg1, preg1);
-    if (c0 < c1) commit(c0, b0, b0 + HEAD_PBUF, qreg0, preg0);
+    uint32_t mA = tmask16(c0), mB = tmask16(c0 + 1), mC = tmask16(c0 + 2), mD = tmask16(c0 + 3);
+    issue(c0, mA, qreg0, preg0);
+    issue(c0 + 1, mB, qreg1, preg1);
+    if (c0 < c1 && mA != 0u) commit(c0, b0, b0 + HEAD_PBUF, qreg0, preg0);
     __syncthreads();
     for (int c = c0; c < c1; c += 2) {
-        issue(c + 2, qreg0, preg0);
-        if (active) compute(b0, b0 + HEAD_PBUF);
-        if (c + 1 < c1) commit(c + 1, b1, b1 + HEAD_PBUF, qreg1, preg1);
+        const uint32_t mE = tmask16(c + 4), mF = tmask16(c + 5);
+        issue(c + 2, mC, qreg0, preg0);
+        if (active && mA != 0u) compute(b0, b0 + HEAD_PBUF);
+        if (c + 1 < c1 && mB != 0u) commit(c + 1, b1, b1 + HEAD_PBUF, qreg1, preg1);
         __syncthreads();
         if (c + 1 < c1) {
-            issue(c + 3, qreg1, preg1);
-            if (active) compute(b1, b1 + HEAD_PBUF);
-            if (c + 2 < c1) commit(c + 2, b0, b0 + HEAD_PBUF, qreg0, preg0);
+            issue(c + 3, mD, qreg1, preg1);
+            if (active && mB != 0u) compute(b1, b1 + HEAD_PBUF);
+            if (c + 2 < c1 && mC != 0u) commit(c + 2, b0, b0 + HEAD_PBUF, qreg0, preg0);
             __syncthreads();
         }
+        mA = mC; mB = mD; mC = mE; mD = mF;
     }
     if (BLK && a.rowsum != nullptr) {
 #pragma unroll
@@ -236,7 +246,7 @@
     k.nchunks = d->B * k.HW / 128; k.nsplit = d->nsplit; k.mtiles = abc_cdiv(d->Ca, 32); k.Ca_pad = k.mtiles * 32;
     k.drop_p = d->q.drop_p; k.drop_seed = d->q.drop_seed; k.drop_salt = d->q.drop_salt;
     k.bytesP = (unsigned)((int64_t)d->B * d->Ca * k.HW * 4); k.bytesQ = (unsigned)((int64_t)d->B * k.HW * d->q.ldx * 2);
-    k.cpad_blk = 0; k.keep = nullptr;
+    k.cpad_blk = 0; k.keep = nullptr; k.tiles = nullptr;
 }
 
 static bool head_dims_ok(const abc_wgrad_desc* d) { return d->p.Hx == d->Hg && d->p.Wx == d->Wg && d->q.Hx == d->Hg && d->q.Wx == d->Wg; }
@@ -382,6 +392,7 @@
             k.bytesP = (unsigned)((size_t)nchunk * cpad * 128 * 2); k.bytesQ = (unsigned)((int64_t)d->B * HW * d->ld * 2);
             k.cpad_blk = cpad;
             k.keep = d->keep_mask != nullptr ? (const uint8_t*)d->keep_mask + (size_t)(i - 5) * nchunk * 2048 : nullptr;
+            k.tiles = i == 5 ? d->dl_tiles : nullptr;
             if ((size_t)nchunk * cpad * 128 * 2 >= (size_t(1) << 31)) return abc_fail(ABC_EUNSUPPORTED, "heads_fused_wgrad: d(logits) block above 2 GB");
             rk.partial[i] = k.partial; rk.rowsum[i] = k.rowsum;
         }
diff --git a/abc-net_amd/engine.py b/abc-net_amd/engine.py
--- a/abc-net_amd/engine.py
+++ b/abc-net_amd/engine.py
@@ -109,7 +109,7 @@
     def __init__(self, variant, in_channels, heads, params, grads, buffers, counters, layout, B, H, W, dtype, train,
                  dropout_p=0.2, device="cuda", drop_seed=0x1234ABCD, fold_bn=False, fused_heads=False, batched_heads=True, fp8=False,
                  guards=False, heads_epilogue=False, actbwd_epilogue=True, merge_reduce=True, nms_heads=False, decode=False,
-                 dual_wgrad=True, fused_convt=True):
+                 dual_wgrad=True, fused_convt=True, zero_skip=True):
         if variant not in ("unet", "unet2"):
             raise NotImplementedError("variant %r" % variant)
         if H < 32 or W < 32:
@@ -141,6 +141,7 @@
         self.btype_idx = None
         self.actbwd_epilogue = bool(actbwd_epilogue)
         self.merge_reduce = bool(merge_reduce)
+        self.zero_skip = bool(zero_skip)
         self._pending_reduce = None
         self.dt = L.BF16 if dtype == "bf16" else L.F32
         self.tdt = torch.bfloat16 if dtype == "bf16" else torch.float32
@@ -908,6 +909,9 @@
         if self.drop_p > 0:
             self.hf_keep = self.new((3 * B * h * w * 16,), torch.uint8, 0)
             d.keep_mask = self.hf_keep.data_ptr()
+        self.hf_tiles = self.new((nchunk,), torch.int64, 0)
+        d.dl_tiles = self.hf_tiles.data_ptr()
+        d.no_zero_skip = 0 if self.zero_skip else 1
         for i in range(nh):
             p = "out_modules.%d.conv2" % i
             d.w2[i], d.b2[i], d.logits[i] = self.P(p + ".weight"), self.P(p + ".bias"), self.logits[i].data_ptr()
diff --git a/abc-net_amd/model.py b/abc-net_amd/model.py
--- a/abc-net_amd/model.py
+++ b/abc-net_amd/model.py
@@ -226,7 +226,7 @@
         return super().load_state_dict(state_dict, strict=strict)
 
     def _engine_for(self, x, train, fold_bn=False, fused_heads=False, batched_heads=True, fp8=False, guards=False, heads_epilogue=False,
-                    actbwd_epilogue=True, merge_reduce=True, nms_heads=False, decode=False, dual_wgrad=True, fused_convt=True):
+                    actbwd_epilogue=True, merge_reduce=True, nms_heads=False, decode=False, dual_wgrad=True, fused_convt=True, zero_skip=True):
         if not x.is_cuda:
             raise L.AbcNetHipError("abcnet_amd runs on an MI355X only (got a %s tensor); there is no CPU fallback" % x.device)
         if x.device != self._flat.device:
@@ -237,7 +237,7 @@
         if Cc != self.n_channels:
             raise ValueError("expected %d input channels, got %d" % (self.n_channels, Cc))
         key = (B, H, W, bool(train), self.compute_dtype, self.dropout_seed, bool(fold_bn), bool(fused_heads), bool(batched_heads), bool(fp8), bool(guards), bool(heads_epilogue), bool(actbwd_epilogue), bool(merge_reduce),
-               bool(nms_heads), bool(decode), bool(dual_wgrad), bool(fused_convt), L.load().abc_get_reserved_cus())
+               bool(nms_heads), bool(decode), bool(dual_wgrad), bool(fused_convt), bool(zero_skip), L.load().abc_get_reserved_cus())
         eng = self._engines.get(key)
         if eng is None or eng.params.data_ptr() != self._flat.data_ptr():
             if self._flat_grad is None or self._flat_grad.device != x.device:
@@ -249,7 +249,7 @@
                              self._counters, (self._lay_p, self._lay_b, self._lay_c), B, H, W, self.compute_dtype, train,
                              dropout_p=self.dropout_p, device=x.device, drop_seed=self.dropout_seed, fold_bn=fold_bn,
                              fused_heads=fused_heads, batched_heads=batched_heads, fp8=fp8, guards=guards, heads_epilogue=heads_epilogue, nms_heads=nms_heads,
-                             actbwd_epilogue=actbwd_epilogue, merge_reduce=merge_reduce, decode=decode, dual_wgrad=dual_wgrad, fused_convt=fused_convt)
+                             actbwd_epilogue=actbwd_epilogue, merge_reduce=merge_reduce, decode=decode, dual_wgrad=dual_wgrad, fused_convt=fused_convt, zero_skip=zero_skip)
             self._engines[key] = eng
         return eng
 
diff --git a/abc-net_amd/train.py b/abc-net_amd/train.py
--- a/abc-net_amd/train.py
+++ b/abc-net_amd/train.py
@@ -14,7 +14,7 @@
     def __init__(self, model, batch, height, width, lr=2.5e-4, weight_decay=1e-8, use_graph=True, bucket_mb=8.0,
                  process_group=None, device=None, metrics=False, broadcast_buffers="lazy", fused_heads=True, keep_logits=True,
                  batched_heads=True, exchange="all_reduce", force_exchange=False, guards=False, actbwd_epilogue=True, merge_reduce=True,
-                 reserve_cus=None, dual_wgrad=True, fused_convt=True, exchange_dtype="f32"):
+                 reserve_cus=None, dual_wgrad=True, fused_convt=True, exchange_dtype="f32", zero_skip=True):
         if exchange_dtype not in D.GradReducer.WIRE_DTYPES:
             raise ValueError("Trainer: exchange_dtype must be one of %s, got %r" % (D.GradReducer.WIRE_DTYPES, exchange_dtype))
         if exchange_dtype == "bf16" and exchange != "direct":
@@ -39,7 +39,7 @@
         with torch.cuda.device(dev):
             x0 = torch.zeros((batch, model.n_channels, height, width), device=dev)
             self.eng = model._engine_for(x0, True, fused_heads=fused_heads, batched_heads=batched_heads, guards=guards,
-                                         actbwd_epilogue=actbwd_epilogue, merge_reduce=merge_reduce, dual_wgrad=dual_wgrad, fused_convt=fused_convt)
+                                         actbwd_epilogue=actbwd_epilogue, merge_reduce=merge_reduce, dual_wgrad=dual_wgrad, fused_convt=fused_convt, zero_skip=zero_skip)
         eng = self.eng
         self.targets = alloc_targets(batch, eng.h, eng.w, dev)
         off_s, _ = model._lay_p["s"]
diff --git a/include/abcnet_hip.h b/include/abcnet_hip.h
--- a/include/abcnet_hip.h
+++ b/include/abcnet_hip.h
@@ -277,6 +277,7 @@
     float* wgrad_work;
     void* keep_mask;
     const uint32_t* target_flags; const void* zero_bytes;
+    uint64_t* dl_tiles; int32_t no_zero_skip; int32_t pad_;
 } abc_heads_fused_desc;
 int64_t abc_heads_fused_pack_bytes(void);
 int abc_heads_fused_chunks(const abc_heads_fused_desc* d);
```

Measured after the change: 2925 images/sec (median of 6 runs). +1.6%, better.
